# lbcb-sci/GNNome

Hardware: AMD Instinct MI355X
Metric: edges/sec full-graph GatedGCN fwd (higher is better)
Workload: dtype f32

## Files before the change

### gnnome_amd/_lib.py

```python
import ctypes
import os

_HERE = os.path.dirname(os.path.abspath(__file__))
LIB_PATH = os.environ.get("GNNOME_HIP_LIB") or os.path.join(_HERE, "lib", "libgnnome_hip.so")
HEADER_PATH = os.path.join(os.path.dirname(_HERE), "include", "gnnome_hip.h")

_p = ctypes.c_void_p
_i = ctypes.c_int
_l = ctypes.c_int64
_sz = ctypes.c_size_t

SIGNATURES = {
    "gnnome_abi_version": [],
    "gnnome_last_error": [],
    "gnnome_set_tuning": [_i, _i],
    "gnnome_debug_gate_profile": [_p],
    "gnnome_graph_views_workspace_bytes": [_l, _l, ctypes.POINTER(_sz)],
    "gnnome_build_graph_views": [_p, _p, _l, _l, _p, _p, _p, _p, _p, _p, _p, _p, _sz, _p],
    "gnnome_encode_f32": [_p, _l, _i, _p, _p, _p, _i, _p, _p, _i, _p, _p],
    "gnnome_linear_f32": [_p, _l, _i, _i, _p, _i, _p, _i, _p, _i, _p],
    "gnnome_linear_acc_f32": [_p, _l, _i, _i, _p, _i, _p, _i, _p, _i, _p],
    "gnnome_weight_planes_f16": [_p, _i, _i, _i, _p, _p],
    "gnnome_linear_planes_f32": [_p, _l, _i, _i, _p, _p, _i, _p, _i, _p],
    "gnnome_linear_planes_route": [_l, _i, _i, _i],
    "gnnome_edge_gate_f32": [_p, _p, _l, _i, _p, _p, _i, _p, _p, _p, _i, _i, _p, _p, _p],
    "gnnome_edge_gate_encode_f32": [_p, _p, _p, _p, _p, _p, _p, _l, _i, _p, _p, _i, _p, _p, _p, _i, _p, _p, _p],
    "gnnome_linear_ref_f32": [_p, _l, _i, _i, _p, _i, _p, _i, _p, _i, _p],
    "gnnome_edge_gate_ref_f32": [_p, _p, _l, _i, _p, _p, _i, _p, _p, _p, _i, _p, _p, _p, _p, _p, _p, _p, _p, _p, _p],
    "gnnome_node_aggregate_f32": [_p, _i, _l, _p, _p, _p, _i, _p, _p, _p, _p, _p, _p, _i, _p, _i, _p, _p, _p],
    "gnnome_build_node_records": [_p, _p, _p, _p, _p, _l, _p, _p],
    "gnnome_debug_node_records": [_p],
    "gnnome_node_aggregate_range_f32": [_p, _i, _l, _l, _l, _p, _p, _p, _i, _p, _p, _p, _p, _p, _p, _i, _p, _i, _p, _p, _p],
    "gnnome_stream_schedule_sizes": [_l, _l, _i, ctypes.POINTER(_l), ctypes.POINTER(_sz)],
    "gnnome_build_stream_schedule": [_l, _l, _p, _p, _p, _p, _p, _i, _i, _i, _p, _p, _p, _p, _p, _p, _p, _p, _sz, _p],
    "gnnome_node_aggregate_stream_f32": [_p, _i, _l, _l, _p, _p, _p, _i, _p, _p, _p, _p, _p, _p, _i, _p, _p, _p, _i, _i, _i, _p, _p, _p, _p, _p, _p,
                                         _p, _l, _p, _p],
    "gnnome_edge_score_f32": [_p, _l, _i, _i, _p, _p, _i, _p, _p, _p, _p, _i, _p, _p, _p, _p, _p, _p, _p],
    "gnnome_debug_forward_events": [_p, _p, _p, _p, _i],
    "gnnome_model_forward_workspace_bytes": [_l, _l, _i, _i, ctypes.POINTER(_sz)],
    "gnnome_model_forward_f32": [_p, _p, _p, _p, _p, _p, _sz, _p],
    "gnnome_model_forward_buffers_f32": [_p, _p, _p, _p, _p, _p, _p],
    "gnnome_edge_gate_raw_f32": [_p, _p, _l, _i, _p, _p, _i, _p, _p, _p, _i, _p],
    "gnnome_edge_gate_raw_stats_rows": [_i, ctypes.POINTER(_i)],
    "gnnome_edge_gate_raw_stats_f32": [_p, _p, _l, _i, _p, _p, _i, _p, _p, _p, _i, _p, _p, _p],
    "gnnome_edge_gate_raw_stats_x16": [_p, _p, _l, _i, _p, _p, _i, _p, _p, _p, _i, _p, _p, _p],
    "gnnome_edge_gate_bn_f32": [_p, _p, _p, _l, _i, _p, _p, _i, _p, _p, _p, _i, _p, _p, _p],
    "gnnome_edge_gate_bn_x16": [_p, _p, _p, _l, _i, _p, _p, _i, _p, _p, _p, _i, _p, _p, _p],
    "gnnome_node_aggregate_raw_f32": [_p, _i, _l, _i, _p, _p, _p, _i, _p, _p, _p, _p, _p, _p, _p, _p, _p, _p, _p],
    "gnnome_colsum_workspace_bytes": [ctypes.POINTER(_sz)],
    "gnnome_colsum2_f32": [_p, _p, _l, _i, _p, _p, _p, _p, _sz, _p],
    "gnnome_bn_relu_res_f32": [_p, _p, _p, _p, _l, _i, _p, _p],
    "gnnome_bn_relu_res_x16": [_p, _p, _p, _p, _l, _i, _p, _p],
    "gnnome_bn_bwd_stats_f32": [_p, _p, _p, _p, _p, _l, _i, _p, _p, _p, _sz, _p],
    "gnnome_bn_bwd_apply_f32": [_p, _p, _p, _p, _l, _i, _p, _p, _p, _p, _p, _p, _p],
    "gnnome_bn_bwd_apply_tables_f32": [_p, _p, _p, _p, _l, _i, _p, _p, _p, _p, _p, _p, _p, _p, _p, _p, _p, _p, _p, _p, _p, _p],
    "gnnome_ln_relu_res_f32": [_p, _p, _p, _p, _l, _i, _i, _p, _p],
    "gnnome_ln_bwd_f32": [_p, _p, _p, _p, _l, _i, _i, _p, _p, _p, _p, _sz, _p],
    "gnnome_mul23_f32": [_p, _p, _p, _l, _p, _p, _p],
    "gnnome_add_f32": [_p, _p, _l, _p, _p],
    "gnnome_relu_bwd_f32": [_p, _p, _l, _p, _p],
    "gnnome_segment_sum_f32": [_p, _i, _p, _p, _l, _p, _i, _p],
    "gnnome_segment_sum2_f32": [_p, _i, _p, _p, _p, _l, _p, _i, _p, _i, _p],
    "gnnome_segment_sum2_amax_f32": [_p, _i, _p, _p, _p, _l, _p, _i, _p, _i, _p, _p],
    "gnnome_segment_sum2_x16": [_p, _i, _p, _p, _p, _l, _p, _i, _p, _i, _p],
    "gnnome_wgrad_workspace_bytes": [_l, _i, _i, ctypes.POINTER(_sz)],
    "gnnome_wgrad_f32": [_p, _i, _i, _p, _i, _i, _l, _p, _i, _p, _sz, _p],
    "gnnome_wgrad_scaled_f32": [_p, _i, _i, _p, _i, _i, _l, _p, _p, _i, _p, _sz, _p],
    "gnnome_wgrad_x16": [_p, _i, _i, _p, _i, _i, _l, _p, _i, _p, _sz, _p],
    "gnnome_wgrad_blocks_f32": [_p, _i, _i, _i, _p, _i, _i, _l, _p, _i, _p, _p, _sz, _p],
    "gnnome_wgrad_blocks_scaled_f32": [_p, _i, _i, _i, _p, _i, _i, _l, _p, _p, _i, _p, _p, _sz, _p],
    "gnnome_linear_blocks_f32": [_p, _i, _i, _l, _i, _p, _i, _i, _p, _i, _i, _p],
    "gnnome_linear_blocks_scaled_f32": [_p, _i, _i, _l, _i, _p, _i, _i, _p, _p, _i, _i, _p],
    "gnnome_score_tail_bwd_f32": [_p, _p, _p, _l, _i, _p, _p, _p, _p, _p, _p, _p],
    "gnnome_agg_edge_bwd_f32": [_p, _l, _i, _p, _p, _p, _p, _p, _p, _i, _p, _p, _p, _p],
    "gnnome_encode_hidden_f32": [_p, _l, _i, _p, _p, _p, _i, _p, _p],
    "gnnome_gather_rows_f32": [_p, _i, _p, _l, _i, _p, _i, _p],
    "gnnome_scatter_add_rows_f32": [_p, _i, _p, _l, _i, _p, _i, _p],
    "gnnome_closure_workspace_bytes": [ctypes.POINTER(_sz)],
    "gnnome_degree_features_f32": [_p, _p, _l, _i, _p, _p, _sz, _p],
    "gnnome_edge_features_f32": [_p, _p, _l, _p, _p, _sz, _p],
    "gnnome_bn_bwd_dgrad_f32": [_p, _p, _l, _l, _i, _p, _p, _p, _p, _p, _p, _p, _p, _i, _p, _p],
    "gnnome_bn_bwd_dgrad_amax_f32": [_p, _p, _l, _l, _i, _p, _p, _p, _p, _p, _p, _p, _p, _i, _p, _p, _p],
    "gnnome_bn_bwd_dgrad_out_f32": [_p, _p, _p, _l, _l, _i, _p, _p, _p, _p, _p, _p, _p, _p, _i, _p, _p],
    "gnnome_bn_bwd_dgrad_out_amax_f32": [_p, _p, _p, _l, _l, _i, _p, _p, _p, _p, _p, _p, _p, _p, _i, _p, _p, _p],
    "gnnome_bn_bwd_dgrad_x16": [_p, _p, _l, _l, _i, _p, _p, _p, _p, _p, _p, _p, _p, _i, _p, _p],
    "gnnome_bn_bwd_dgrad_out_x16": [_p, _p, _p, _l, _l, _i, _p, _p, _p, _p, _p, _p, _p, _p, _i, _p, _p],
    "gnnome_agg_edge_bwd_stats_f32": [_p, _l, _i, _p, _p, _p, _p, _p, _p, _i, _p, _p, _p, _p, _p, _p, _p, _p, _p, _p, _sz, _p],
    "gnnome_agg_edge_bwd_stats_x16": [_p, _l, _i, _p, _p, _p, _p, _p, _p, _i, _p, _p, _p, _p, _p, _p, _p, _p, _p, _p, _sz, _p],
    "gnnome_agg_bwd_fused_f32": [_p, _l, _l, _i, _p, _p, _p, _p, _p, _p, _i, _p, _p, _p, _p, _p, _p, _p, _p, _p, _p, _p, _p, _p, _p, _p, _p, _sz, _p],
    "gnnome_agg_bwd_fused_x16": [_p, _l, _l, _i, _p, _p, _p, _p, _p, _p, _i, _p, _p, _p, _p, _p, _p, _p, _p, _p, _p, _p, _p, _p, _p, _p, _p, _sz, _p],
    "gnnome_bn_bwd_terms_f32": [_p, _p, _p, _l, _i, _p, _p, _p, _p],
    "gnnome_pack_layer_f32": [_p, _p, _p, _p, _i, _p, _p, _p, _p, _p],
    "gnnome_bn_train_finish_f32": [_p, _p, _p, _l, _i, _p, _p, _p, _p, _p, ctypes.c_float, ctypes.c_float, _i, _p, _p, _p, _p, _p],
    "gnnome_gate_center_f32": [_p, _l, _i, _p, _p, _i, _p, _p, _p, _i, _p, _p],
    "gnnome_greedy_walks_workspace_bytes": [_l, _i, ctypes.POINTER(_sz)],
    "gnnome_greedy_walks": [_p, _p, _p, _p, _p, _p, _p, _l, _p, _p, _p, _i, _p, _p, _l, _p, _p, _p, _p, _p, _p, _p, _sz, _p],
    "gnnome_mark_walk_visited": [_p, _p, _p, _l, _p, _p],
    "gnnome_overlap_workspace_bytes": [ctypes.POINTER(_sz)],
    "gnnome_overlap_edit_distance": [_p, _p, _l, _p, _i, _p, _p, _p, _l, _p, _p, _p, _sz, _p],
    "gnnome_contig_pieces_workspace_bytes": [_l, _l, ctypes.POINTER(_sz)],
    "gnnome_contig_pieces": [_p, _l, _p, _l, _p, _p, _p, _p, _l, _p, _l, _p, _p, _sz, _p],
    "gnnome_contig_spell": [_p, _l, _p, _l, _p, _p, _p, _l, _p, _i, _p, _l, _p],
    "gnnome_edge_labels_workspace_bytes": [_l, _l, ctypes.POINTER(_sz)],
    "gnnome_edge_labels": [_p, _p, _l, _l, _p, _p, _p, _p, _p, _p, _l, _p, _sz, _p],
    "gnnome_cluster_inputs_workspace_bytes": [_l, _l, ctypes.POINTER(_sz)],
    "gnnome_cluster_inputs_f32": [_p, _p, _l, _l, _p, _p, _l, _p, _l, _p, _l, _p, _p, _l, _p, _p, _l, _p, _p, _p, _p, _p, _sz, _p],
    "gnnome_adjacency_support": [_p, _p, _p, _l, _l, _p, _p],
    "gnnome_bfs_levels": [_p, _p, _l, _p, _p, _p, _p, _p, _p, _p],
    "gnnome_hem_propose": [_p, _p, _p, _p, _p, _l, _i, _p, _p],
    "gnnome_kway_gains": [_p, _p, _p, _p, _l, _p, _p, _p],
    "gnnome_greedy_growing_host": [_p, _p, _p, _p, _l, _i, _p],
    "gnnome_edge_loss_f32": [_p, _p, _p, _l, _p, ctypes.c_float, ctypes.c_float, _p, _p, _p, _p, _p, _sz, _p],
    "gnnome_gfa_tile_sizes": [ctypes.POINTER(_i), ctypes.POINTER(_i)],
    "gnnome_gfa_mark": [_p, _l, _p, _p, _p],
    "gnnome_gfa_classify": [_p, _l, _p, _p, _l, _p, _l, _p, _p, _p, _p, _p],
    "gnnome_gfa_names_insert": [_p, _l, _p, _p, _l, _p, _l, _p, _l, _p, _p],
    "gnnome_gfa_links": [_p, _l, _p, _p, _l, _p, _p, _l, _p, _l, _p, _l, _p, _p, _p, _p],
    "gnnome_gfa_pack": [_p, _l, _p, _p, _l, _p, _l, _p],
}

ABI_VERSION = 21


class LayerParams(ctypes.Structure):
    _fields_ = [(n, _p) for n in ("Wcat", "Wcat_planes", "bcat", "W3", "b3", "scale_e", "shift_e", "scale_h", "shift_h")] + [
        ("norm_kind", ctypes.c_int32), ("reference_order", ctypes.c_int32)]


class ModelParams(ctypes.Structure):
    _fields_ = ([(n, ctypes.c_int32) for n in ("hidden", "hidden_ne", "num_layers", "score_hidden", "node_features", "edge_features")]
                + [(n, _p) for n in ("node_W1", "node_b1", "node_W2", "node_b2", "edge_W1", "edge_b1", "edge_W2", "edge_b2")]
                + [("layers_host", ctypes.POINTER(LayerParams)), ("W_nodes", _p), ("W_nodes_planes", _p), ("b_nodes", _p), ("W1e", _p),
                   ("ld_w1e", ctypes.c_int32), ("reserved", ctypes.c_int32), ("W2", _p), ("b2", _p), ("W3", _p), ("b3", _p)])


class Views(ctypes.Structure):
    _fields_ = ([("num_nodes", ctypes.c_int64), ("num_edges", ctypes.c_int64)]
                + [(n, _p) for n in ("in_ptr", "srt_src", "srt_dst", "srt_eid", "out_ptr", "out_pos", "out_dst", "node_gather")]
                + [("transposed", ctypes.c_int32), ("reserved", ctypes.c_int32)])


class ForwardBuffers(ctypes.Structure):
    _fields_ = [("h", _p * 2), ("P", _p), ("e", _p * 2), ("PQ", _p)]


NORM_AFFINE = 0
NORM_LAYER = 1

_lib = None


class GnnomeHipError(RuntimeError):
    pass


def load():
    global _lib
    if _lib is not None:
        return _lib
    if not os.path.isfile(LIB_PATH):
        raise GnnomeHipError(
            f"{LIB_PATH} not found - the HIP extension is not built. Run `make -C gnnome_amd/csrc` "
            "(or __graft_entry__.build()). gnnome_amd has no CPU fallback.")
    lib = ctypes.CDLL(LIB_PATH)
    for name, argtypes in SIGNATURES.items():
        fn = getattr(lib, name)
        fn.argtypes = argtypes
        fn.restype = ctypes.c_char_p if name == "gnnome_last_error" else _i
    got = lib.gnnome_abi_version()
    if got != ABI_VERSION:
        raise GnnomeHipError(f"libgnnome_hip.so ABI {got} != binding ABI {ABI_VERSION}; rebuild")
    _lib = lib
    return lib


def check(rc, what):
    if rc != 0:
        msg = load().gnnome_last_error()
        raise GnnomeHipError(f"{what} failed ({rc}): {msg.decode() if msg else ''}")
```

### gnnome_amd/csrc/common.h

```cpp
#pragma once
#include <hip/hip_runtime.h>
#include <stdint.h>
#include <stdio.h>

#include "../../include/gnnome_hip.h"

namespace gnnome {

void set_error(const char* fmt, ...);

enum { kTuneGateVariant = 0, kTuneGateAblation = 1, kTuneLinearVariant = 2, kTuneGateTileOrder = 3, kTuneGateExperiment = 4, kTuneAggLdsKiB = 5, kTuneAggHubs = 6, kTuneAggVariant = 7, kTuneRefVariant = 8, kTuneOverlapBand = 9, kTuneArith = 10, kTuneCount = 16 };
int tuning(int key);

struct GateEnc {
    const float* e_raw;
    const int32_t* srt_eid;
    const float *W1, *b1, *W2, *b2;
    const float *W23, *b23;
};

struct GateBnBwd {
    const float *a, *c1, *c2, *mean, *rstd, *scale, *shift;
    float* a_out;
    int64_t n_once;
    unsigned* amax_bits = nullptr;
};

struct GateBfArgs {
    const float* e_in;
    float* e_out;
    int64_t E;
    const float* B1h;
    const float* B2h;
    int ldn;
    const int32_t* srt_src;
    const int32_t* srt_dst;
    const float* W3;
    int ldw;
    const float* scale;
    const float* shift;
    float* stats;
    int num_tiles;
    int abl;
    long long* prof;
    int xp;
    int num_cblocks, ld_out;
    GateEnc enc;
    GateBnBwd bnb;
};
int gate_bf_launch(int hidden, int mode, bool enc, const GateBfArgs& args, hipStream_t s, bool x16 = false, int extra = 0);
int gate_stream_launch(const float* e_in, float* e_out, int64_t E, const float* B1h, const float* B2h, int ldn, const int32_t* ss,
                       const int32_t* sd, const float* W3, int ldw, const float* scale, const float* shift, hipStream_t s);

int ws_linear_acc(const float* A, int64_t M, int K, const float* W, int ldw, float* C, hipStream_t s);
int stream_linear_acc_256(const float* A, int64_t M, const float* W, int ldw, float* C, hipStream_t s);
int gate_pl256_launch(int mode, const GateBfArgs& a, hipStream_t s, bool x16 = false);
int gate_f16_launch(int mode, const GateBfArgs& a, int grid, hipStream_t s, bool x16 = false);
int gate_enc256_launch(const GateBfArgs& a, hipStream_t s);
int gate_pl256_stats_rows();
void hub_cache_invalidate();
long long* gate_profile_buffer();
int linear_refm_launch(const float* A, int64_t M, int K, int lda, const float* W, int ldw, const float* bias, int Nout, float* C, int ldc,
                       hipStream_t s);
int gate_refm_launch(int hidden, bool with_enc, const float* e_in, float* e_out, int64_t E, const float* B1h, const float* B2h, int ldn,
                     const int32_t* ss, const int32_t* sd, const float* W3, int ldw, const float* b3, const float* scale, const float* shift,
                     const GateEnc& enc, hipStream_t s);

#define GN_REQUIRE(cond, ...)                 \
    do {                                      \
        if (!(cond)) {                        \
            ::gnnome::set_error(__VA_ARGS__); \
            return GNNOME_EINVAL;             \
        }                                     \
    } while (0)

#define GN_HIP(call)                                                                              \
    do {                                                                                          \
        hipError_t err__ = (call);                                                                \
        if (err__ != hipSuccess) {                                                                \
            ::gnnome::set_error("%s failed: %s (%s:%d)", #call, hipGetErrorString(err__), __FILE__, \
                                __LINE__);                                                        \
            return GNNOME_EHIP;                                                                   \
        }                                                                                         \
    } while (0)

#define GN_LAUNCH_CHECK() GN_HIP(hipGetLastError())

constexpr int kWave = 64;
constexpr int kXcds = 8;
constexpr int kNumCUs = 256;
int persistent_grid();
constexpr float kAggEps = 1e-6f;
constexpr float kNormEps = 1e-5f;

typedef float f32x4 __attribute__((ext_vector_type(4)));
typedef float f32x16 __attribute__((ext_vector_type(16)));

__device__ __forceinline__ unsigned bf16_bits(float x) {
    const unsigned u = __float_as_uint(x);
    return (u + 0x7FFFu + ((u >> 16) & 1u)) >> 16;
}
__device__ __forceinline__ uint2 pack_bf16x4(const f32x4 v) {
    return make_uint2(bf16_bits(v[0]) | (bf16_bits(v[1]) << 16), bf16_bits(v[2]) | (bf16_bits(v[3]) << 16));
}
__device__ __forceinline__ f32x4 unpack_bf16x4(const uint2 p) {
    return f32x4{__uint_as_float(p.x << 16), __uint_as_float(p.x & 0xFFFF0000u), __uint_as_float(p.y << 16),
                 __uint_as_float(p.y & 0xFFFF0000u)};
}
template <bool X16>
__device__ __forceinline__ f32x4 load4_as(const void* base, int64_t off) {
    if (X16) return unpack_bf16x4(*reinterpret_cast<const uint2*>(reinterpret_cast<const uint16_t*>(base) + off));
    return *reinterpret_cast<const f32x4*>(reinterpret_cast<const float*>(base) + off);
}
template <bool X16>
__device__ __forceinline__ void store4_as(void* base, int64_t off, const f32x4 v) {
    if (X16)
        *reinterpret_cast<uint2*>(reinterpret_cast<uint16_t*>(base) + off) = pack_bf16x4(v);
    else
        *reinterpret_cast<f32x4*>(reinterpret_cast<float*>(base) + off) = v;
}


__device__ __forceinline__ int xcd_remap(int bid, int n) {
    const int xcd = bid % kXcds, q = n / kXcds, r = n % kXcds;
    const int base = xcd < r ? xcd * (q + 1) : r * (q + 1) + (xcd - r) * q;
    return base + bid / kXcds;
}

__device__ __forceinline__ float sigmoidf_(float x) { return __builtin_amdgcn_rcpf(1.0f + __expf(-x)); }

__device__ __forceinline__ float relu_keep_nan(float t) { return t < 0.f ? 0.f : t; }

__device__ __forceinline__ void wave_amax_to(unsigned* amax_bits, float v) {
#pragma unroll
    for (int o = 32; o > 0; o >>= 1) v = fmaxf(v, __shfl_xor(v, o));
    if ((threadIdx.x & 63) == 0) {
        const unsigned b = __float_as_uint(v);
        if (b > __hip_atomic_load(amax_bits, __ATOMIC_RELAXED, __HIP_MEMORY_SCOPE_AGENT)) atomicMax(amax_bits, b);
    }
}

__device__ __forceinline__ float half_wave_sum(float v) {
    v += __shfl_xor(v, 1);
    v += __shfl_xor(v, 2);
    v += __shfl_xor(v, 4);
    v += __shfl_xor(v, 8);
    v += __shfl_xor(v, 16);
    return v;
}

}
```

### gnnome_amd/csrc/edge_gate.hip

```cpp
#include "gemm_tile.h"

namespace gnnome {

template <int NB, int NORM>
__global__ __launch_bounds__(kGemmThreads) void k_edge_gate(const float* e_in, float* e_out, int64_t E,
                                                            const float* __restrict__ B1h,
                                                            const float* __restrict__ B2h, int ldn,
                                                            const int32_t* __restrict__ srt_src,
                                                            const int32_t* __restrict__ srt_dst,
                                                            const float* __restrict__ W3, int ldw,
                                                            const float* __restrict__ scale,
                                                            const float* __restrict__ shift, int total_tiles, int norm_width) {
    constexpr int H = 32 * NB;
    __shared__ __attribute__((aligned(16))) float lds[tile_lds_floats<NB>() + 2 * kTileM];
    float* As = lds;
    float* Ws = lds + kTileM * kLdk;
    int* s_src = reinterpret_cast<int*>(lds + tile_lds_floats<NB>());
    int* s_dst = s_src + kTileM;

    const int tid = threadIdx.x, wave = tid >> 6, lane = tid & 63;
    const int tile = xcd_remap(blockIdx.x, total_tiles);
    const int64_t row0 = (int64_t)tile * kTileM;
    const int valid = (int)min((int64_t)kTileM, E - row0);

// ... 489 lines not shown
               "edge_gate: null pointer");
    const int norm_width = (norm_kind >> 8) ? (norm_kind >> 8) : hidden;
    norm_kind &= 0xFF;
    GN_REQUIRE(norm_kind == GNNOME_NORM_AFFINE || norm_kind == GNNOME_NORM_LAYER, "edge_gate: bad norm_kind %d", norm_kind);
    GN_REQUIRE(norm_width >= 1 && norm_width <= hidden && (norm_width == hidden || norm_kind == GNNOME_NORM_LAYER), "edge_gate: bad norm width %d", norm_width);
    GN_REQUIRE(ld_node >= hidden && ldw >= hidden && ldw % 4 == 0, "edge_gate: bad strides");
    GN_REQUIRE(((uintptr_t)e_in % 16 == 0) && ((uintptr_t)W3 % 16 == 0), "edge_gate: e_in and W3 must be 16-byte aligned");
    hipStream_t s = (hipStream_t)stream;
    const int variant = tuning(kTuneGateVariant);
    const bool rows16 = ld_node % 4 == 0 && ((uintptr_t)B1h % 16 == 0) && ((uintptr_t)B2h % 16 == 0);
    const bool persistent_ok = norm_kind == GNNOME_NORM_AFFINE && (hidden == 64 || hidden == 128);
    if (persistent_ok && variant != 1) {
        if ((variant == 0 || variant == 7 || variant == 8) && rows16) {
            GateBfArgs a = {};
            a.e_in = e_in; a.e_out = e_out; a.E = num_edges; a.B1h = B1h; a.B2h = B2h; a.ldn = ld_node; a.srt_src = srt_src;
            a.srt_dst = srt_dst; a.W3 = W3; a.ldw = ldw; a.scale = norm_scale; a.shift = norm_shift;
            return gate_bf_launch(hidden, 0, false, a, s);
        }
        if ((variant == 5 || variant == 6) && rows16) {
            if (hidden == 128)
                return launch_gate_ws<4, 1>(e_in, e_out, num_edges, B1h, B2h, ld_node, srt_src, srt_dst, W3, ldw, norm_scale, norm_shift, s);
            return launch_gate_ws<2, 2>(e_in, e_out, num_edges, B1h, B2h, ld_node, srt_src, srt_dst, W3, ldw, norm_scale, norm_shift, s);
        }
    }
    if (hidden == 256 && norm_kind == GNNOME_NORM_AFFINE && (variant == 0 || variant == 9) && e_in != e_out && ld_node % 4 == 0 &&
        ((uintptr_t)e_out % 16 == 0)) {
        if (variant == 0 && rows16) {
            GateBfArgs a = {};
            a.e_in = e_in; a.e_out = e_out; a.E = num_edges; a.B1h = B1h; a.B2h = B2h; a.ldn = ld_node; a.srt_src = srt_src;
            a.srt_dst = srt_dst; a.W3 = W3; a.ldw = ldw; a.scale = norm_scale; a.shift = norm_shift;
            return gate_pl256_launch(0, a, s);
        }
        return gate_stream_launch(e_in, e_out, num_edges, B1h, B2h, ld_node, srt_src, srt_dst, W3, ldw, norm_scale, norm_shift, s);
    }
    switch (hidden) {
        case 64: return launch_gate<2>(e_in, e_out, num_edges, B1h, B2h, ld_node, srt_src, srt_dst, W3, ldw, norm_kind, norm_scale, norm_shift, s, norm_width);
        case 128: return launch_gate<4>(e_in, e_out, num_edges, B1h, B2h, ld_node, srt_src, srt_dst, W3, ldw, norm_kind, norm_scale, norm_shift, s, norm_width);
        case 256: return launch_gate<8>(e_in, e_out, num_edges, B1h, B2h, ld_node, srt_src, srt_dst, W3, ldw, norm_kind, norm_scale, norm_shift, s, norm_width);
        default: set_error("edge_gate: hidden=%d not in {64,128,256}", hidden); return GNNOME_EINVAL;
    }
}

extern "C" int gnnome_edge_gate_raw_f32(const float* e_in, float* x_out, int64_t num_edges, int hidden, const float* B1h,
                                        const float* B2h, int ld_node, const int32_t* srt_src, const int32_t* srt_dst,
                                        const float* W3, int ldw, void* stream) {
    using namespace gnnome;
    GN_REQUIRE(num_edges >= 0, "edge_gate_raw: negative edge count");
    if (num_edges == 0) return GNNOME_OK;
    GN_REQUIRE(e_in && x_out && x_out != e_in && B1h && B2h && srt_src && srt_dst && W3, "edge_gate_raw: bad pointers");
    GN_REQUIRE(ld_node >= hidden && ldw >= hidden && ldw % 4 == 0, "edge_gate_raw: bad strides");
    GN_REQUIRE(((uintptr_t)e_in % 16 == 0) && ((uintptr_t)W3 % 16 == 0), "edge_gate_raw: e_in and W3 must be 16-byte aligned");
    hipStream_t s = (hipStream_t)stream;
    if (hidden == 256 && tuning(kTuneGateVariant) == 0 && ld_node % 4 == 0 && ((uintptr_t)B1h % 16 == 0) && ((uintptr_t)B2h % 16 == 0) &&
        ((uintptr_t)x_out % 16 == 0)) {
        GateBfArgs a = {};
        a.e_in = e_in; a.e_out = x_out; a.E = num_edges; a.B1h = B1h; a.B2h = B2h; a.ldn = ld_node; a.srt_src = srt_src;
        a.srt_dst = srt_dst; a.W3 = W3; a.ldw = ldw;
        return gate_pl256_launch(1, a, s);
    }
    switch (hidden) {
        case 64: return launch_gate<2>(e_in, x_out, num_edges, B1h, B2h, ld_node, srt_src, srt_dst, W3, ldw, 2, nullptr, nullptr, s);
        case 128: return launch_gate<4>(e_in, x_out, num_edges, B1h, B2h, ld_node, srt_src, srt_dst, W3, ldw, 2, nullptr, nullptr, s);
        case 256: return launch_gate<8>(e_in, x_out, num_edges, B1h, B2h, ld_node, srt_src, srt_dst, W3, ldw, 2, nullptr, nullptr, s);
        default: set_error("edge_gate_raw: hidden=%d not in {64,128,256}", hidden); return GNNOME_EINVAL;
    }
}

extern "C" int gnnome_edge_gate_raw_stats_rows(int hidden, int* rows_host) {
    using namespace gnnome;
    GN_REQUIRE(rows_host && (hidden == 64 || hidden == 128 || hidden == 256), "edge_gate_raw_stats_rows: hidden=%d not in {64,128,256}", hidden);
    if (hidden == 256) {
        *rows_host = gate_pl256_stats_rows();
        return GNNOME_OK;
    }
    *rows_host = (tuning(kTuneGateVariant) == 0 || tuning(kTuneGateVariant) == 8) ? kNumCUs * 8 : kNumCUs * (hidden == 128 ? 1 : 2);
    return GNNOME_OK;
}

static int raw_stats_impl(const float* e_in, void* x_out, int64_t num_edges, int hidden, const float* B1h,
                          const float* B2h, int ld_node, const int32_t* srt_src, const int32_t* srt_dst,
                          const float* W3, int ldw, const float* center, float* stats_partial, void* stream, bool x16) {
    using namespace gnnome;
    GN_REQUIRE(num_edges > 0, "edge_gate_raw_stats: needs at least one edge");
    GN_REQUIRE(e_in && x_out != (const void*)e_in && B1h && B2h && srt_src && srt_dst && W3 && center && stats_partial,
               "edge_gate_raw_stats: bad pointers");
    GN_REQUIRE(x_out || ((hidden == 128 || (hidden == 256 && tuning(kTuneArith) == 0 && !x16)) && tuning(kTuneGateVariant) == 0),
               "edge_gate_raw_stats: x_out may be NULL at hidden = 128 and, as fp16x3 with fp32 storage, 256 (default kernels)");
    GN_REQUIRE(hidden == 64 || hidden == 128 || hidden == 256, "edge_gate_raw_stats: hidden=%d not in {64,128,256}", hidden);
    GN_REQUIRE(ld_node >= hidden && ld_node % 4 == 0 && ldw >= hidden && ldw % 4 == 0, "edge_gate_raw_stats: bad strides");
    GN_REQUIRE(((uintptr_t)e_in % 16 == 0) && ((uintptr_t)W3 % 16 == 0) && ((uintptr_t)B1h % 16 == 0) && ((uintptr_t)B2h % 16 == 0),
               "edge_gate_raw_stats: 16-byte alignment required");
    hipStream_t s = (hipStream_t)stream;
    if (hidden == 256) {
        GateBfArgs a = {};
        a.e_in = e_in; a.e_out = (float*)x_out; a.E = num_edges; a.B1h = B1h; a.B2h = B2h; a.ldn = ld_node; a.srt_src = srt_src;
        a.srt_dst = srt_dst; a.W3 = W3; a.ldw = ldw; a.scale = center; a.stats = stats_partial;
        return gate_pl256_launch(1, a, s, x16);
    }
    if (tuning(kTuneGateVariant) == 0 || tuning(kTuneGateVariant) == 8 || x16) {
        GateBfArgs a = {};
        a.e_in = e_in; a.e_out = (float*)x_out; a.E = num_edges; a.B1h = B1h; a.B2h = B2h; a.ldn = ld_node; a.srt_src = srt_src;
        a.srt_dst = srt_dst; a.W3 = W3; a.ldw = ldw; a.scale = center; a.stats = stats_partial;
        return gate_bf_launch(hidden, 1, false, a, s, x16, x_out == nullptr ? 1 : 0);
    }
    if (hidden == 128)
        return launch_ws_raw_stats<4, 1>(e_in, (float*)x_out, num_edges, B1h, B2h, ld_node, srt_src, srt_dst, W3, ldw, center, stats_partial, s);
    return launch_ws_raw_stats<2, 2>(e_in, (float*)x_out, num_edges, B1h, B2h, ld_node, srt_src, srt_dst, W3, ldw, center, stats_partial, s);
}

extern "C" int gnnome_edge_gate_raw_stats_f32(const float* e_in, float* x_out, int64_t num_edges, int hidden, const float* B1h,
                                              const float* B2h, int ld_node, const int32_t* srt_src, const int32_t* srt_dst,
                                              const float* W3, int ldw, const float* center, float* stats_partial, void* stream) {
    return raw_stats_impl(e_in, x_out, num_edges, hidden, B1h, B2h, ld_node, srt_src, srt_dst, W3, ldw, center, stats_partial, stream, false);
}

extern "C" int gnnome_edge_gate_raw_stats_x16(const float* e_in, uint16_t* x_out, int64_t num_edges, int hidden, const float* B1h,
                                              const float* B2h, int ld_node, const int32_t* srt_src, const int32_t* srt_dst,
                                              const float* W3, int ldw, const float* center, float* stats_partial, void* stream) {
    return raw_stats_impl(e_in, x_out, num_edges, hidden, B1h, B2h, ld_node, srt_src, srt_dst, W3, ldw, center, stats_partial, stream, true);
}

static int gate_bn_impl(const float* e_in, float* e_out, void* x_out, int64_t num_edges, int hidden, const float* B1h, const float* B2h, int ld_node,
                        const int32_t* srt_src, const int32_t* srt_dst, const float* W3, int ldw, const float* scale, const float* shift,
                        void* stream, bool x16) {
    using namespace gnnome;
    GN_REQUIRE(num_edges >= 0, "edge_gate_bn: negative edge count");
    if (num_edges == 0) return GNNOME_OK;
    GN_REQUIRE(e_in && e_out && x_out && x_out != (const void*)e_in && x_out != (void*)e_out && B1h && B2h && srt_src && srt_dst && W3 && scale && shift,
               "edge_gate_bn: bad pointers");
    GN_REQUIRE((hidden == 128 || (hidden == 256 && tuning(kTuneArith) == 0 && !x16)) && tuning(kTuneGateVariant) == 0,
               "edge_gate_bn: built at hidden = 128 and, as fp16x3 with fp32 storage, 256 (default kernels), got %d", hidden);
    GN_REQUIRE(ld_node >= hidden && ld_node % 4 == 0 && ldw >= hidden && ldw % 4 == 0, "edge_gate_bn: bad strides");
    GN_REQUIRE(((uintptr_t)e_in % 16 == 0) && ((uintptr_t)e_out % 16 == 0) && ((uintptr_t)x_out % 16 == 0) && ((uintptr_t)W3 % 16 == 0) &&
                   ((uintptr_t)B1h % 16 == 0) && ((uintptr_t)B2h % 16 == 0), "edge_gate_bn: 16-byte alignment required");
    GateBfArgs a = {};
    a.e_in = e_in; a.e_out = e_out; a.E = num_edges; a.B1h = B1h; a.B2h = B2h; a.ldn = ld_node; a.srt_src = srt_src; a.srt_dst = srt_dst;
    a.W3 = W3; a.ldw = ldw; a.scale = scale; a.shift = shift; a.bnb.a_out = (float*)x_out;
    if (hidden == 256) return gate_pl256_launch(0, a, (hipStream_t)stream, false);
    return gate_bf_launch(hidden, 0, false, a, (hipStream_t)stream, x16, 1);
}

extern "C" int gnnome_edge_gate_bn_f32(const float* e_in, float* e_out, float* x_out, int64_t num_edges, int hidden, const float* B1h,
                                       const float* B2h, int ld_node, const int32_t* srt_src, const int32_t* srt_dst, const float* W3, int ldw,
                                       const float* scale, const float* shift, void* stream) {
    return gate_bn_impl(e_in, e_out, x_out, num_edges, hidden, B1h, B2h, ld_node, srt_src, srt_dst, W3, ldw, scale, shift, stream, false);
}

extern "C" int gnnome_edge_gate_bn_x16(const float* e_in, float* e_out, uint16_t* x_out, int64_t num_edges, int hidden, const float* B1h,
                                       const float* B2h, int ld_node, const int32_t* srt_src, const int32_t* srt_dst, const float* W3, int ldw,
                                       const float* scale, const float* shift, void* stream) {
    return gate_bn_impl(e_in, e_out, x_out, num_edges, hidden, B1h, B2h, ld_node, srt_src, srt_dst, W3, ldw, scale, shift, stream, true);
}

extern "C" int gnnome_edge_gate_encode_f32(const float* e_raw, const int32_t* srt_eid, const float* encW1, const float* encb1,
                                           const float* encW2, const float* encb2, float* e_out, int64_t num_edges, int hidden,
                                           const float* B1h, const float* B2h, int ld_node, const int32_t* srt_src,
                                           const int32_t* srt_dst, const float* W3, int ldw, const float* norm_scale,
                                           const float* norm_shift, void* stream) {
    using namespace gnnome;
    GN_REQUIRE(num_edges >= 0, "edge_gate_encode: negative edge count");
    if (num_edges == 0) return GNNOME_OK;
    GN_REQUIRE(e_raw && srt_eid && encW1 && encb1 && encW2 && encb2 && e_out && B1h && B2h && srt_src && srt_dst && W3 &&
                   norm_scale && norm_shift, "edge_gate_encode: null pointer");
    GN_REQUIRE(hidden == 64 || hidden == 128 || (hidden == 256 && tuning(kTuneArith) == 0 && tuning(kTuneGateVariant) == 0),
               "edge_gate_encode: hidden=%d not in {64,128,256 (default kernels)}", hidden);
    GN_REQUIRE(ld_node % 4 == 0 && ldw % 4 == 0 && ((uintptr_t)B1h % 16 == 0) && ((uintptr_t)B2h % 16 == 0) && ((uintptr_t)W3 % 16 == 0),
               "edge_gate_encode: alignment");
    const GateEnc enc = {e_raw, srt_eid, encW1, encb1, encW2, encb2};
    hipStream_t s = (hipStream_t)stream;
    if (hidden == 256) {
        GN_REQUIRE((uintptr_t)e_out % 16 == 0, "edge_gate_encode: e_out must be 16-byte aligned");
        GateBfArgs a = {};
        a.e_out = e_out; a.E = num_edges; a.B1h = B1h; a.B2h = B2h; a.ldn = ld_node; a.srt_src = srt_src; a.srt_dst = srt_dst;
        a.W3 = W3; a.ldw = ldw; a.scale = norm_scale; a.shift = norm_shift; a.enc = enc;
        return gate_enc256_launch(a, s);
    }
    if (tuning(kTuneGateVariant) == 0 || tuning(kTuneGateVariant) == 7 || tuning(kTuneGateVariant) == 8) {
        GateBfArgs a = {};
        a.e_out = e_out; a.E = num_edges; a.B1h = B1h; a.B2h = B2h; a.ldn = ld_node; a.srt_src = srt_src; a.srt_dst = srt_dst;
        a.W3 = W3; a.ldw = ldw; a.scale = norm_scale; a.shift = norm_shift; a.enc = enc;
        return gate_bf_launch(hidden, 0, true, a, s);
    }
    if (hidden == 128)
        return launch_gate_ws<4, 1>(nullptr, e_out, num_edges, B1h, B2h, ld_node, srt_src, srt_dst, W3, ldw, norm_scale, norm_shift, s, &enc);
    return launch_gate_ws<2, 2>(nullptr, e_out, num_edges, B1h, B2h, ld_node, srt_src, srt_dst, W3, ldw, norm_scale, norm_shift, s, &enc);
}
```

### gnnome_amd/csrc/edge_gate_bf.hip

```cpp
#include "common.h"

namespace gnnome {

typedef __bf16 bf16x8 __attribute__((ext_vector_type(8)));

template <int CB, int RB>
struct GateBF {
    static_assert(CB * RB == 4, "four compute waves");
    static constexpr int H = 32 * CB, TM = 32 * RB, LDK = H + 4, RING = 4, LWAVES = 2;
    static constexpr int NT = 64 * (4 + RING * LWAVES);
    static constexpr int NP = TM * (H / 4) / (64 * LWAVES);
    static constexpr int kSlotFloats = TM * LDK;
    static constexpr int kLdsFloats = RING * 2 * kSlotFloats;
};

__device__ __forceinline__ unsigned lds_addr_bf(const void* p) {
    return (unsigned)(size_t)(__attribute__((address_space(3))) const void*)p;
}
__device__ __forceinline__ void flag_wait_bf(unsigned addr, unsigned want, int nap) {
    unsigned v, spins = 0;
    for (;;) {
        asm volatile("ds_read_b32 %0, %1\n\ts_waitcnt lgkmcnt(0)" : "=v"(v) : "v"(addr) : "memory");
        if (__builtin_amdgcn_readfirstlane(v) >= want) break;
        if (++spins > (1u << 26)) __builtin_trap();
// ... 747 lines not shown
    constexpr int H = 128, TM = 32, RING = 3, LDK = H + 4, TPLD = 48, TPLANE = TM * TPLD, TILEF = TM * LDK;
    constexpr int SLOTB = 3 * TPLANE + 2 * TILEF * 4, NP = 8, RSTEP = 4;
    __shared__ __attribute__((aligned(16))) unsigned char ring[RING * SLOTB];
    __shared__ __attribute__((aligned(16))) float consts[4 * H];
    __shared__ float w1s[32], b1s[16];
    __shared__ unsigned flags[2 * RING];
    const int tid = threadIdx.x, lane = tid & 63;
    const int wave = __builtin_amdgcn_readfirstlane(tid >> 6);
    const unsigned full0 = lds_addr_bf(&flags[0]), done0 = lds_addr_bf(&flags[RING]);
    const int per_xcd = gridDim.x / kXcds;
    const int first = (int)(blockIdx.x % kXcds) * per_xcd + (int)(blockIdx.x / kXcds);
    const int stride = (int)gridDim.x;
    const int n = first < a.num_tiles ? (a.num_tiles - first + stride - 1) / stride : 0;
    if (n <= 0) return;
    auto tile_of = [&](int r) { return first + r * stride; };
    auto tile_valid = [&](int r) { return (int)min((int64_t)TM, a.E - (int64_t)tile_of(r) * TM); };
    if (tid < 4 * H) {
        const int q = tid / H, c = tid % H;
        consts[tid] = q == 0 ? a.scale[c] : q == 1 ? a.shift[c] : q == 2 ? a.enc.b23[c] : a.enc.b2[c];
    }
    if (tid >= 4 * H && tid < 4 * H + 32) w1s[tid - 4 * H] = a.enc.W1[tid - 4 * H];
    if (tid >= 4 * H + 32 && tid < 4 * H + 48) b1s[tid - 4 * H - 32] = a.enc.b1[tid - 4 * H - 32];
    if (tid < 2 * RING) flags[tid] = 0;
    __syncthreads();

    if (wave < 4) {
        const int cl = lane & 31, half = lane >> 5, col = 32 * wave + cl;
        uint4 u1, u2, u3, v1, v2, v3;
        {
            const float* p = a.enc.W23 + col * 16 + 8 * half;
            split3(*reinterpret_cast<const f32x4*>(p), *reinterpret_cast<const f32x4*>(p + 4), u1, u2, u3);
            const float* q = a.enc.W2 + col * 16 + 8 * half;
            split3(*reinterpret_cast<const f32x4*>(q), *reinterpret_cast<const f32x4*>(q + 4), v1, v2, v3);
        }
        auto crow = [](int r) { return (r & 3) + 8 * (r >> 2); };
        const int lane_x = 4 * half * LDK + col;
        const float bxc = consts[2 * H + col], bec = consts[3 * H + col];
        for (int i = 0; i < n; ++i) {
            const int slot = i % RING;
            const unsigned use = (unsigned)(i / RING) + 1u;
            flag_wait_bf(full0 + 4 * slot, 2u * use, 0);
            const unsigned char* tp = ring + slot * SLOTB + cl * TPLD + 16 * half;
            const uint4 c1 = *reinterpret_cast<const uint4*>(tp), c2 = *reinterpret_cast<const uint4*>(tp + TPLANE),
                        c3 = *reinterpret_cast<const uint4*>(tp + 2 * TPLANE);
            f32x16 ax, ae;
#pragma unroll
            for (int r = 0; r < 16; ++r) ax[r] = ae[r] = 0.f;
            ax = __builtin_amdgcn_mfma_f32_32x32x16_bf16(as_bf(c3), as_bf(u1), ax, 0, 0, 0);
            ae = __builtin_amdgcn_mfma_f32_32x32x16_bf16(as_bf(c3), as_bf(v1), ae, 0, 0, 0);
            ax = __builtin_amdgcn_mfma_f32_32x32x16_bf16(as_bf(c1), as_bf(u3), ax, 0, 0, 0);
            ae = __builtin_amdgcn_mfma_f32_32x32x16_bf16(as_bf(c1), as_bf(v3), ae, 0, 0, 0);
            ax = __builtin_amdgcn_mfma_f32_32x32x16_bf16(as_bf(c2), as_bf(u2), ax, 0, 0, 0);
            ae = __builtin_amdgcn_mfma_f32_32x32x16_bf16(as_bf(c2), as_bf(v2), ae, 0, 0, 0);
            ax = __builtin_amdgcn_mfma_f32_32x32x16_bf16(as_bf(c2), as_bf(u1), ax, 0, 0, 0);
            ae = __builtin_amdgcn_mfma_f32_32x32x16_bf16(as_bf(c2), as_bf(v1), ae, 0, 0, 0);
            ax = __builtin_amdgcn_mfma_f32_32x32x16_bf16(as_bf(c1), as_bf(u2), ax, 0, 0, 0);
            ae = __builtin_amdgcn_mfma_f32_32x32x16_bf16(as_bf(c1), as_bf(v2), ae, 0, 0, 0);
            ax = __builtin_amdgcn_mfma_f32_32x32x16_bf16(as_bf(c1), as_bf(u1), ax, 0, 0, 0);
            ae = __builtin_amdgcn_mfma_f32_32x32x16_bf16(as_bf(c1), as_bf(v1), ae, 0, 0, 0);
            float* X = reinterpret_cast<float*>(ring + slot * SLOTB + 3 * TPLANE) + lane_x;
#pragma unroll
            for (int r = 0; r < 16; ++r) {
                X[crow(r) * LDK] = ax[r] + bxc;
                X[TILEF + crow(r) * LDK] = ae[r] + bec;
            }
            flag_bump_bf(done0 + 4 * slot, lane);
        }
    } else {
        const int group = (wave - 4) / 2;
        const int gl = ((wave - 4) % 2) * 64 + lane;
        const int r0 = gl / (H / 4), c4 = gl % (H / 4);
        const int trow = gl >> 2, jq = gl & 3;
        f32x4 g1[NP], g2[NP], gk[NP];
        int si[NP], di[NP], eid = 0;
        float raw0 = 0.f, raw1 = 0.f;
        const unsigned off_row = (unsigned)(r0 * H + 4 * c4);
        auto issue_early = [&](int r) {
            const int64_t row0 = (int64_t)tile_of(r) * TM;
            const int valid = tile_valid(r);
#pragma unroll
            for (int p = 0; p < NP; ++p) {
                const int64_t row = row0 + min(r0 + p * RSTEP, valid - 1);
                si[p] = a.srt_src[row];
                di[p] = a.srt_dst[row];
            }
            eid = a.enc.srt_eid[row0 + min(trow, valid - 1)];
        };
        auto issue_late = [&]() {
            raw0 = a.enc.e_raw[2 * (int64_t)eid];
            raw1 = a.enc.e_raw[2 * (int64_t)eid + 1];
#pragma unroll
            for (int p = 0; p < NP; ++p) {
                g1[p] = *reinterpret_cast<const f32x4*>(a.B1h + (int64_t)si[p] * a.ldn + 4 * c4);
                g2[p] = *reinterpret_cast<const f32x4*>(a.B2h + (int64_t)di[p] * a.ldn + 4 * c4);
            }
        };
        if (group < n) {
            issue_early(group);
            issue_late();
            if (group + RING < n) issue_early(group + RING);
        }
        unsigned char* S = ring + group * SLOTB;
        const float* Xs = reinterpret_cast<const float*>(S + 3 * TPLANE);
        for (int r = group; r < n; r += RING) {
            const unsigned use = (unsigned)(r / RING) + 1u;
            {
                f32x4 t;
#pragma unroll
                for (int j = 0; j < 4; ++j) {
                    const int hu = 4 * jq + j;
                    t[j] = fmaxf(__builtin_fmaf(raw1, w1s[2 * hu + 1], raw0 * w1s[2 * hu]) + b1s[hu], 0.f);
                }
                uint2 p1, p2, p3;
                split4_planes(t, p1, p2, p3);
                unsigned char* d = S + trow * TPLD + 8 * jq;
                *reinterpret_cast<uint2*>(d) = p1;
                *reinterpret_cast<uint2*>(d + TPLANE) = p2;
                *reinterpret_cast<uint2*>(d + 2 * TPLANE) = p3;
            }
#pragma unroll
            for (int p = 0; p < NP; ++p) {
                gk[p] = g1[p] + g2[p];
                asm volatile("" : "+v"(gk[p]));
            }
            flag_bump_bf(full0 + 4 * group, lane);
            if (r + RING < n) issue_late();
            if (r + 2 * RING < n) issue_early(r + 2 * RING);
            flag_wait_bf(done0 + 4 * group, 4u * use, a.xp & 3);
            const int valid = tile_valid(r);
            const f32x4 sc4 = *reinterpret_cast<const f32x4*>(consts + 4 * c4), sh4 = *reinterpret_cast<const f32x4*>(consts + H + 4 * c4);
            float* out = a.e_out + (int64_t)tile_of(r) * TM * H;
#pragma unroll
            for (int pb = 0; pb < NP; pb += 2) {
                f32x4 x[2], e0[2];
#pragma unroll
                for (int u = 0; u < 2; ++u) {
                    x[u] = *reinterpret_cast<const f32x4*>(Xs + (r0 + (pb + u) * RSTEP) * LDK + 4 * c4);
                    e0[u] = *reinterpret_cast<const f32x4*>(Xs + TILEF + (r0 + (pb + u) * RSTEP) * LDK + 4 * c4);
                }
                asm volatile("" : "+v"(x[0]), "+v"(x[1]));
#pragma unroll
                for (int u = 0; u < 2; ++u) {
                    const int p = pb + u, row = r0 + p * RSTEP;
                    f32x4 y;
#pragma unroll
                    for (int j = 0; j < 4; ++j) y[j] = fmaxf((x[u][j] + gk[p][j]) * sc4[j] + sh4[j], 0.f) + e0[u][j];
                    if (row < valid) *reinterpret_cast<f32x4*>(out + (off_row + (unsigned)(p * RSTEP * H))) = y;
                }
            }
        }
    }
}

struct EncFoldScratch {
    float* w23 = nullptr;
};
static EncFoldScratch g_enc_fold[16];

static int launch_enc16(const GateBfArgs& args, hipStream_t s) {
    GateBfArgs a = args;
    const int64_t tiles = (a.E + 31) / 32;
    GN_REQUIRE(tiles < (1ll << 31), "edge_gate: too many tiles");
    a.num_tiles = (int)tiles;
    a.xp = tuning(kTuneGateExperiment);
    int dev = 0;
    GN_HIP(hipGetDevice(&dev));
    GN_REQUIRE(dev >= 0 && dev < 16, "edge_gate_encode: device index %d", dev);
    if (!g_enc_fold[dev].w23) GN_HIP(hipMalloc(&g_enc_fold[dev].w23, sizeof(float) * (128 * 16 + 128)));
    float* w23 = g_enc_fold[dev].w23;
    hipLaunchKernelGGL(k_fold_encoder, dim3((128 * 17 + 3) / 4), dim3(256), 0, s, a.W3, a.ldw, a.enc.W2, a.enc.b2, 128, w23, w23 + 128 * 16);
    GN_LAUNCH_CHECK();
    a.enc.W23 = w23;
    a.enc.b23 = w23 + 128 * 16;
    hipLaunchKernelGGL(k_edge_gate_enc16, dim3(persistent_grid()), dim3(640), 0, s, a);
    GN_LAUNCH_CHECK();
    return GNNOME_OK;
}

static EncFoldScratch g_enc_fold256[16];
int gate_enc256_launch(const GateBfArgs& args, hipStream_t s) {
    GateBfArgs a = args;
    const int64_t tiles = (a.E + 31) / 32;
    GN_REQUIRE(tiles < (1ll << 31), "edge_gate: too many tiles");
    a.num_tiles = (int)tiles;
    a.prof = g_gate_prof;
    int dev = 0;
    GN_HIP(hipGetDevice(&dev));
    GN_REQUIRE(dev >= 0 && dev < 16, "edge_gate_encode: device index %d", dev);
    if (!g_enc_fold256[dev].w23) GN_HIP(hipMalloc(&g_enc_fold256[dev].w23, sizeof(float) * (256 * 16 + 256)));
    float* w23 = g_enc_fold256[dev].w23;
    hipLaunchKernelGGL(k_fold_encoder, dim3((256 * 17 + 3) / 4), dim3(256), 0, s, a.W3, a.ldw, a.enc.W2, a.enc.b2, 256, w23, w23 + 256 * 16);
    GN_LAUNCH_CHECK();
    a.enc.W23 = w23;
    a.enc.b23 = w23 + 256 * 16;
    int g = persistent_grid();
    g -= g % 16;
    return gate_f16_launch(5, a, g < 16 ? 16 : g, s);
}

template <int CB, int RB, int MODE, bool ENC, bool X16 = false>
static int launch_bf(const GateBfArgs& args, hipStream_t s) {
    using P = GateBF<CB, RB>;
    GateBfArgs a = args;
    const int64_t tiles = (a.E + P::TM - 1) / P::TM;
    GN_REQUIRE(tiles < (1ll << 31), "edge_gate: too many tiles");
    a.num_tiles = (int)tiles;
    a.abl = tuning(kTuneGateAblation);
    a.xp = tuning(kTuneGateExperiment);
    a.prof = g_gate_prof;
    if (MODE == 1) GN_HIP(hipMemsetAsync(a.stats, 0, sizeof(float) * kNumCUs * P::RING * P::LWAVES * 2 * P::H, s));
    hipLaunchKernelGGL((k_edge_gate_bf<CB, RB, MODE, ENC, X16>), dim3(persistent_grid()), dim3(P::NT), 0, s, a);
    GN_LAUNCH_CHECK();
    return GNNOME_OK;
}

int gate_bf_launch(int hidden, int mode, bool enc, const GateBfArgs& a, hipStream_t s, bool x16, int extra) {
    const bool planes = hidden == 128 && tuning(kTuneGateVariant) != 8;
    if (extra) {
        GN_REQUIRE(hidden == 128 && !enc && (mode == 0 || mode == 1), "edge-tile kernel: the two-pass training forward is built at hidden = 128");
        if (mode == 1) return x16 ? launch_pl<false, 1, true, 1>(a, s) : launch_pl<false, 1, false, 1>(a, s);
        return x16 ? launch_pl<false, 0, true, 1>(a, s) : launch_pl<false, 0, false, 1>(a, s);
    }
    if (x16) {
        if (mode == 1 && planes) return launch_pl<false, 1, true>(a, s);
        if (mode == 3 && planes) return launch_pl<false, 3, true>(a, s);
        if (mode == 1) return hidden == 128 ? launch_bf<4, 1, 1, false, true>(a, s) : launch_bf<2, 2, 1, false, true>(a, s);
        if (mode == 3) return hidden == 128 ? launch_bf<4, 1, 3, false, true>(a, s) : launch_bf<2, 2, 3, false, true>(a, s);
        set_error("edge-tile kernel: bf16 storage exists for modes 1 and 3 only");
        return GNNOME_EINVAL;
    }
    if (hidden == 128) {
        if (mode == 0 && enc && tuning(kTuneGateVariant) == 0) return launch_enc16(a, s);
        if (mode == 0 && tuning(kTuneGateVariant) != 8) return enc ? launch_pl<true>(a, s) : launch_pl<false>(a, s);
        if (mode == 1 && planes) return launch_pl<false, 1>(a, s);
        if (mode == 3 && planes) return launch_pl<false, 3>(a, s);
        if (mode == 4) return launch_pl<false, 4>(a, s);
        if (mode == 2 && planes) return launch_pl<false, 2>(a, s);
        if (mode == 0) return enc ? launch_bf<4, 1, 0, true>(a, s) : launch_bf<4, 1, 0, false>(a, s);
        if (mode == 3) return launch_bf<4, 1, 3, false>(a, s);
        return mode == 1 ? launch_bf<4, 1, 1, false>(a, s) : launch_bf<4, 1, 2, false>(a, s);
    }
    if (mode == 0) return enc ? launch_bf<2, 2, 0, true>(a, s) : launch_bf<2, 2, 0, false>(a, s);
    if (mode == 3) return launch_bf<2, 2, 3, false>(a, s);
    return mode == 1 ? launch_bf<2, 2, 1, false>(a, s) : launch_bf<2, 2, 2, false>(a, s);
}

}

extern "C" int gnnome_debug_gate_profile(void* counters) {
    gnnome::g_gate_prof = (long long*)counters;
    return GNNOME_OK;
}

static int bn_bwd_dgrad_impl(float* C, const void* X, int64_t rows, int64_t rows_once, int hidden, const float* scale, const float* shift,
                             const float* a, const float* c1, const float* c2, const float* mean, const float* rstd,
                             const float* W, int ldw, void* dxe, void* stream, bool x16, unsigned* amax_bits = nullptr) {
    using namespace gnnome;
    GN_REQUIRE(rows >= 0 && (hidden == 64 || hidden == 128), "bn_bwd_dgrad: hidden=%d not in {64,128}", hidden);
    GN_REQUIRE(rows_once >= 0 && rows_once <= rows, "bn_bwd_dgrad: rows_once=%lld outside [0, rows]", (long long)rows_once);
    if (rows == 0) return GNNOME_OK;
    GN_REQUIRE(C && X && scale && shift && a && c1 && c2 && mean && rstd && W && dxe && dxe != (void*)C && ldw >= hidden && ldw % 4 == 0,
               "bn_bwd_dgrad: bad arguments");
    GN_REQUIRE(((uintptr_t)C % 16 == 0) && ((uintptr_t)X % 16 == 0) && ((uintptr_t)dxe % 16 == 0) && ((uintptr_t)W % 16 == 0),
               "bn_bwd_dgrad: tensors must be 16-byte aligned");
    GateBfArgs g = {};
    g.e_in = (const float*)X; g.e_out = C; g.E = rows; g.B1h = C; g.ldn = hidden; g.W3 = W; g.ldw = ldw;
    g.bnb = GateBnBwd{a, c1, c2, mean, rstd, scale, shift, (float*)dxe, rows_once};
    if (amax_bits != nullptr) {
        GN_REQUIRE(hidden == 128 && tuning(kTuneGateVariant) != 8, "bn_bwd_dgrad_amax: hidden = 128 on the plane-form kernel only");
        GN_HIP(hipMemsetAsync(amax_bits, 0, sizeof(unsigned), (hipStream_t)stream));
        g.bnb.amax_bits = amax_bits;
    }
    return gate_bf_launch(hidden, 3, false, g, (hipStream_t)stream, x16);
}

extern "C" int gnnome_bn_bwd_dgrad_f32(float* C, const float* X, int64_t rows, int64_t rows_once, int hidden, const float* scale, const float* shift,
                                       const float* a, const float* c1, const float* c2, const float* mean, const float* rstd,
                                       const float* W, int ldw, float* dxe, void* stream) {
    return bn_bwd_dgrad_impl(C, X, rows, rows_once, hidden, scale, shift, a, c1, c2, mean, rstd, W, ldw, dxe, stream, false);
}

extern "C" int gnnome_bn_bwd_dgrad_amax_f32(float* C, const float* X, int64_t rows, int64_t rows_once, int hidden, const float* scale,
                                            const float* shift, const float* a, const float* c1, const float* c2, const float* mean,
                                            const float* rstd, const float* W, int ldw, float* dxe, unsigned* amax_bits, void* stream) {
    GN_REQUIRE(amax_bits != nullptr, "bn_bwd_dgrad_amax: null amax_bits");
    return bn_bwd_dgrad_impl(C, X, rows, rows_once, hidden, scale, shift, a, c1, c2, mean, rstd, W, ldw, dxe, stream, false, amax_bits);
}

extern "C" int gnnome_bn_bwd_dgrad_x16(float* C, const uint16_t* X, int64_t rows, int64_t rows_once, int hidden, const float* scale, const float* shift,
                                       const float* a, const float* c1, const float* c2, const float* mean, const float* rstd,
                                       const float* W, int ldw, uint16_t* dxe, void* stream) {
    return bn_bwd_dgrad_impl(C, X, rows, rows_once, hidden, scale, shift, a, c1, c2, mean, rstd, W, ldw, dxe, stream, true);
}

static int bn_bwd_dgrad_out_impl(const float* C_in, float* C_out, const float* X, int64_t rows, int64_t rows_once, int hidden,
                                 const float* scale, const float* shift, const float* a, const float* c1, const float* c2,
                                 const float* mean, const float* rstd, const float* W, int ldw, float* dxe, void* stream, bool x16,
                                 unsigned* amax_bits = nullptr);
extern "C" int gnnome_bn_bwd_dgrad_out_amax_f32(const float* C_in, float* C_out, const float* X, int64_t rows, int64_t rows_once, int hidden,
                                                const float* scale, const float* shift, const float* a, const float* c1, const float* c2,
                                                const float* mean, const float* rstd, const float* W, int ldw, float* dxe, unsigned* amax_bits,
                                                void* stream) {
    GN_REQUIRE(amax_bits != nullptr, "bn_bwd_dgrad_out_amax: null amax_bits");
    return bn_bwd_dgrad_out_impl(C_in, C_out, X, rows, rows_once, hidden, scale, shift, a, c1, c2, mean, rstd, W, ldw, dxe, stream, false, amax_bits);
}
extern "C" int gnnome_bn_bwd_dgrad_out_f32(const float* C_in, float* C_out, const float* X, int64_t rows, int64_t rows_once, int hidden,
                                           const float* scale, const float* shift, const float* a, const float* c1, const float* c2,
                                           const float* mean, const float* rstd, const float* W, int ldw, float* dxe, void* stream) {
    return bn_bwd_dgrad_out_impl(C_in, C_out, X, rows, rows_once, hidden, scale, shift, a, c1, c2, mean, rstd, W, ldw, dxe, stream, false);
}
extern "C" int gnnome_bn_bwd_dgrad_out_x16(const float* C_in, float* C_out, const uint16_t* X, int64_t rows, int64_t rows_once, int hidden,
                                           const float* scale, const float* shift, const float* a, const float* c1, const float* c2,
                                           const float* mean, const float* rstd, const float* W, int ldw, uint16_t* dxe, void* stream) {
    return bn_bwd_dgrad_out_impl(C_in, C_out, (const float*)X, rows, rows_once, hidden, scale, shift, a, c1, c2, mean, rstd, W, ldw, (float*)dxe, stream, true);
}
static int bn_bwd_dgrad_out_impl(const float* C_in, float* C_out, const float* X, int64_t rows, int64_t rows_once, int hidden,
                                 const float* scale, const float* shift, const float* a, const float* c1, const float* c2,
                                 const float* mean, const float* rstd, const float* W, int ldw, float* dxe, void* stream, bool x16,
                                 unsigned* amax_bits) {
    using namespace gnnome;
    GN_REQUIRE(rows >= 0 && hidden == 256, "bn_bwd_dgrad_out: hidden=%d (256 only; 64 / 128 update C in place: gnnome_bn_bwd_dgrad_f32)", hidden);
    if (amax_bits != nullptr) GN_HIP(hipMemsetAsync(amax_bits, 0, sizeof(unsigned), (hipStream_t)stream));
    GN_REQUIRE(rows_once >= 0 && rows_once <= rows, "bn_bwd_dgrad_out: rows_once=%lld outside [0, rows]", (long long)rows_once);
    if (rows == 0) return GNNOME_OK;
    GN_REQUIRE(C_in && C_out && C_out != C_in && X && scale && shift && a && c1 && c2 && mean && rstd && W && dxe && dxe != C_out && dxe != C_in &&
                   ldw >= hidden && ldw % 4 == 0, "bn_bwd_dgrad_out: bad arguments");
    GN_REQUIRE(((uintptr_t)C_in % 16 == 0) && ((uintptr_t)C_out % 16 == 0) && ((uintptr_t)X % 16 == 0) && ((uintptr_t)dxe % 16 == 0) &&
                   ((uintptr_t)W % 16 == 0), "bn_bwd_dgrad_out: tensors must be 16-byte aligned");
    (void)x16;
    GateBfArgs g = {};
    g.e_in = X; g.e_out = C_out; g.E = rows; g.B1h = C_in; g.ldn = hidden; g.W3 = W; g.ldw = ldw;
    g.bnb = GateBnBwd{a, c1, c2, mean, rstd, scale, shift, dxe, rows_once};
    g.bnb.amax_bits = amax_bits;
    return gate_pl256_launch(3, g, (hipStream_t)stream, x16);
}
```

### gnnome_amd/csrc/model_forward.cpp

```cpp
#include "common.h"

namespace gnnome {
namespace {

constexpr size_t kAlign = 256;
size_t rounded(size_t bytes) { return (bytes + kAlign - 1) / kAlign * kAlign; }

struct Workspace {
    size_t h[2], P, e[2], PQ, total;
};
Workspace layout(int64_t n, int64_t e, int hidden, int hs) {
    Workspace w;
    size_t off = 0;
    auto take = [&](size_t bytes) {
        const size_t at = off;
        off += rounded(bytes);
        return at;
    };
    w.h[0] = take(sizeof(float) * n * hidden);
    w.h[1] = take(sizeof(float) * n * hidden);
    w.P = take(sizeof(float) * n * 5 * hidden);
    w.e[0] = take(sizeof(float) * e * hidden);
    w.e[1] = hidden == 256 ? take(sizeof(float) * e * hidden) : w.e[0];
    w.PQ = take(sizeof(float) * n * 2 * hs);
    w.total = off;
    return w;
}

struct ForwardEvents {
    hipEvent_t ev[4] = {nullptr, nullptr, nullptr, nullptr};
    int layer = -1;
};
thread_local ForwardEvents g_events;
int mark(int which, int layer, void* stream) {
    if (layer != g_events.layer || g_events.ev[which] == nullptr) return GNNOME_OK;
    GN_HIP(hipEventRecord(g_events.ev[which], (hipStream_t)stream));
    return GNNOME_OK;
}

int project(const float* A, int64_t M, int K, const float* W, const void* planes, const float* bias, int Nout, float* C, void* stream) {
    if (planes != nullptr && gnnome_linear_planes_route(M, K, Nout, 1)) return gnnome_linear_planes_f32(A, M, K, K, planes, bias, Nout, C, Nout, stream);
    return gnnome_linear_f32(A, M, K, K, W, K, bias, Nout, C, Nout, stream);
}

}
}

extern "C" int gnnome_debug_forward_events(void* gate_start, void* gate_stop, void* aggregate_start, void* aggregate_stop, int layer) {
    using namespace gnnome;
    g_events.ev[0] = (hipEvent_t)gate_start;
    g_events.ev[1] = (hipEvent_t)gate_stop;
    g_events.ev[2] = (hipEvent_t)aggregate_start;
    g_events.ev[3] = (hipEvent_t)aggregate_stop;
    g_events.layer = layer;
    return GNNOME_OK;
}

extern "C" int gnnome_model_forward_workspace_bytes(int64_t num_nodes, int64_t num_edges, int hidden, int score_hidden, size_t* bytes_host) {
    using namespace gnnome;
    GN_REQUIRE(bytes_host && num_nodes >= 0 && num_edges >= 0 && hidden > 0 && score_hidden > 0, "model_forward_workspace_bytes: bad argument");
    *bytes_host = layout(num_nodes, num_edges, hidden, score_hidden).total;
    return GNNOME_OK;
}

#define GN_TRY(call)                       \
    do {                                   \
        const int rc__ = (call);           \
        if (rc__ != GNNOME_OK) return rc__; \
    } while (0)

namespace gnnome {
namespace {
int forward_on(const gnnome_model_params* m, const gnnome_views* g, const float* x, const float* e_raw, float* logits, float* const h[2], float* P,
               float* const eb[2], float* PQ, void* stream);
}
}

static int check_model(const gnnome_model_params* m, const gnnome_views* g) {
    using namespace gnnome;
    GN_REQUIRE(m && g, "model_forward: null parameter block");
    const int H = m->hidden, hs = m->score_hidden, L = m->num_layers;
    GN_REQUIRE(g->num_nodes >= 0 && g->num_edges >= 0 && L >= 0 && (L == 0 || m->layers_host != nullptr), "model_forward: bad sizes");
    GN_REQUIRE(H == 64 || H == 128 || H == 256, "model_forward: hidden=%d (the kernels are built for 64 / 128 / 256; pad narrower models)", H);
    GN_REQUIRE(hs == 32 || hs == 64 || hs == 128, "model_forward: score_hidden=%d (built for 32 / 64 / 128)", hs);
    return GNNOME_OK;
}

extern "C" int gnnome_model_forward_f32(const gnnome_model_params* m, const gnnome_views* g, const float* x, const float* e_raw, float* logits,
                                        void* workspace, size_t workspace_bytes, void* stream) {
    using namespace gnnome;
    GN_TRY(check_model(m, g));
    const int64_t N = g->num_nodes, E = g->num_edges;
    const Workspace ws = layout(N, E, m->hidden, m->score_hidden);
    if (workspace_bytes < ws.total) {
        set_error("model_forward: workspace of %zu bytes, %zu needed", workspace_bytes, ws.total);
        return GNNOME_EWORKSPACE;
    }
    GN_REQUIRE((N == 0 && E == 0) || (workspace != nullptr && (uintptr_t)workspace % kAlign == 0), "model_forward: workspace must be 256-byte aligned");
    GN_REQUIRE(E == 0 || logits != nullptr, "model_forward: null logits");
    char* base = static_cast<char*>(workspace);
    float* h[2] = {reinterpret_cast<float*>(base + ws.h[0]), reinterpret_cast<float*>(base + ws.h[1])};
    float* eb[2] = {reinterpret_cast<float*>(base + ws.e[0]), reinterpret_cast<float*>(base + ws.e[1])};
    return forward_on(m, g, x, e_raw, logits, h, reinterpret_cast<float*>(base + ws.P), eb, reinterpret_cast<float*>(base + ws.PQ), stream);
}

extern "C" int gnnome_model_forward_buffers_f32(const gnnome_model_params* m, const gnnome_views* g, const float* x, const float* e_raw, float* logits,
                                                const gnnome_forward_buffers* b, void* stream) {
    using namespace gnnome;
    GN_TRY(check_model(m, g));
    GN_REQUIRE(b != nullptr, "model_forward_buffers: null buffer block");
    const int64_t N = g->num_nodes, E = g->num_edges;
    GN_REQUIRE(E == 0 || logits != nullptr, "model_forward_buffers: null logits");
    GN_REQUIRE(N == 0 || (b->h[0] && b->h[1] && b->P && b->PQ && b->h[0] != b->h[1]), "model_forward_buffers: node buffers h[0], h[1], P, PQ");
    GN_REQUIRE(E == 0 || (b->e[0] && (m->hidden != 256 || (b->e[1] && b->e[1] != b->e[0]))), "model_forward_buffers: edge buffers e[0] (and e[1] at hidden = 256)");
    for (const void* p : {(const void*)b->h[0], (const void*)b->h[1], (const void*)b->P, (const void*)b->e[0], (const void*)b->e[1], (const void*)b->PQ})
        GN_REQUIRE((uintptr_t)p % 16 == 0, "model_forward_buffers: buffers must be 16-byte aligned");
    float* h[2] = {b->h[0], b->h[1]};
    float* eb[2] = {b->e[0], m->hidden == 256 ? b->e[1] : b->e[0]};
    return forward_on(m, g, x, e_raw, logits, h, b->P, eb, b->PQ, stream);
}

namespace gnnome {
namespace {
int forward_on(const gnnome_model_params* m, const gnnome_views* g, const float* x, const float* e_raw, float* logits, float* const h[2], float* P,
               float* const eb[2], float* PQ, void* stream) {
    const int64_t N = g->num_nodes, E = g->num_edges;
    const int H = m->hidden, hs = m->score_hidden, L = m->num_layers;

    GN_TRY(gnnome_encode_f32(x, N, m->node_features, g->node_gather, m->node_W1, m->node_b1, m->hidden_ne, m->node_W2, m->node_b2, H, h[0], stream));
    const bool wide_ok = tuning(kTuneArith) == 0 && tuning(kTuneGateVariant) == 0;
    const bool fold = L > 0 && m->edge_features == 2 && m->hidden_ne == 16 && (H == 64 || H == 128 || (H == 256 && wide_ok)) &&
                      m->layers_host[0].norm_kind == GNNOME_NORM_AFFINE && E > 0;
    float* e = nullptr;
    if (!fold) {
        e = eb[0];
        GN_TRY(gnnome_encode_f32(e_raw, E, m->edge_features, g->srt_eid, m->edge_W1, m->edge_b1, m->hidden_ne, m->edge_W2, m->edge_b2, H, e, stream));
    }
    int cur = 0;
    for (int i = 0; i < L; ++i) {
        const gnnome_layer_params& lw = m->layers_host[i];
        if (lw.reference_order) GN_TRY(gnnome_linear_ref_f32(h[cur], N, H, H, lw.Wcat, H, lw.bcat, 5 * H, P, 5 * H, stream));
        else GN_TRY(project(h[cur], N, H, lw.Wcat, lw.Wcat_planes, lw.bcat, 5 * H, P, stream));
        const float *A1 = P, *A2 = P + H, *A3 = P + 2 * H, *B1 = P + 3 * H, *B2 = P + 4 * H;
        if (g->transposed) {
            const float* t = A2; A2 = A3; A3 = t;
            t = B1; B1 = B2; B2 = t;
        }
        GN_TRY(mark(0, i, stream));
        if (lw.reference_order) {
            float* out = e ? e : eb[0];
            GN_TRY(gnnome_edge_gate_ref_f32(e, out, E, H, B1, B2, 5 * H, g->srt_src, g->srt_dst, lw.W3, H, lw.b3, lw.scale_e, lw.shift_e,
                                            e ? nullptr : e_raw, e ? nullptr : g->srt_eid, e ? nullptr : m->edge_W1, e ? nullptr : m->edge_b1,
                                            e ? nullptr : m->edge_W2, e ? nullptr : m->edge_b2, stream));
            e = out;
        } else if (e == nullptr) {
            GN_TRY(gnnome_edge_gate_encode_f32(e_raw, g->srt_eid, m->edge_W1, m->edge_b1, m->edge_W2, m->edge_b2, eb[0], E, H, B1, B2, 5 * H, g->srt_src,
                                               g->srt_dst, lw.W3, H, lw.scale_e, lw.shift_e, stream));
            e = eb[0];
        } else if (H == 256 && lw.norm_kind == GNNOME_NORM_AFFINE) {
            float* out = e == eb[0] ? eb[1] : eb[0];
            GN_TRY(gnnome_edge_gate_f32(e, out, E, H, B1, B2, 5 * H, g->srt_src, g->srt_dst, lw.W3, H, lw.norm_kind, lw.scale_e, lw.shift_e, stream));
            e = out;
        } else {
            GN_TRY(gnnome_edge_gate_f32(e, e, E, H, B1, B2, 5 * H, g->srt_src, g->srt_dst, lw.W3, H, lw.norm_kind, lw.scale_e, lw.shift_e, stream));
        }
        GN_TRY(mark(1, i, stream));
        GN_TRY(mark(2, i, stream));
        GN_TRY(gnnome_node_aggregate_f32(e, H, N, A1, A2, A3, 5 * H, g->in_ptr, g->srt_src, g->out_ptr, g->out_pos, g->out_dst, h[cur], H, h[cur ^ 1],
                                         lw.norm_kind, lw.scale_h, lw.shift_h, stream));
        GN_TRY(mark(3, i, stream));
        cur ^= 1;
    }
    GN_TRY(project(h[cur], N, H, m->W_nodes, m->W_nodes_planes, m->b_nodes, 2 * hs, PQ, stream));
    const float *Ps = PQ, *Qd = PQ + hs;
    if (g->transposed) {
        const float* t = Ps; Ps = Qd; Qd = t;
    }
    return gnnome_edge_score_f32(e, E, H, hs, Ps, Qd, 2 * hs, g->srt_src, g->srt_dst, g->srt_eid, m->W1e, m->ld_w1e, m->W2, m->b2, m->W3, m->b3, logits,
                                 nullptr, stream);
}
}
}
```

### gnnome_amd/csrc/node_project.hip

```cpp
#include <cstdlib>

#include "common.h"

#pragma clang diagnostic ignored "-Winline-asm"

namespace gnnome {
namespace {

typedef _Float16 h2_t __attribute__((ext_vector_type(2)));
typedef _Float16 h8_t __attribute__((ext_vector_type(8)));
typedef float f32x2 __attribute__((ext_vector_type(2)));

constexpr float kLoScale = 2048.f, kLoInv = 1.0f / 2048.f;

__device__ __forceinline__ unsigned lds_addr(const void* p) { return (unsigned)(size_t)(__attribute__((address_space(3))) const void*)p; }

__device__ __forceinline__ void dma_piece(const void* src, unsigned voff, unsigned lds) {
    asm volatile("s_mov_b32 m0, %2\n\ts_nop 0\n\tglobal_load_lds_dwordx4 %0, %1" ::"v"(voff), "s"(src), "s"(lds) : "m0");
}

template <int N>
__device__ __forceinline__ void wait_vm() { asm volatile("s_waitcnt vmcnt(%0)" ::"n"(N) : "memory"); }
template <int OFF>
__device__ __forceinline__ void load16_at(f32x4& dst, const float* p) {
    asm volatile("global_load_dwordx4 %0, %1, off offset:%2" : "=v"(dst) : "v"(p), "n"(OFF) : "memory");
}
__device__ __forceinline__ void load4_raw(float& dst, const float* p) { asm volatile("global_load_dword %0, %1, off" : "=v"(dst) : "v"(p) : "memory"); }
__device__ __forceinline__ void landed8(f32x4* r, bool wait) {
    if (wait)
        asm volatile("s_waitcnt vmcnt(0)" : "+v"(r[0]), "+v"(r[1]), "+v"(r[2]), "+v"(r[3]), "+v"(r[4]), "+v"(r[5]), "+v"(r[6]), "+v"(r[7])::"memory");
    else
        asm volatile("" : "+v"(r[0]), "+v"(r[1]), "+v"(r[2]), "+v"(r[3]), "+v"(r[4]), "+v"(r[5]), "+v"(r[6]), "+v"(r[7])::"memory");
}

__device__ __forceinline__ float quad_xor1(float v) { return __int_as_float(__builtin_amdgcn_mov_dpp(__float_as_int(v), 0xB1, 0xF, 0xF, true)); }
__device__ __forceinline__ float quad_xor2(float v) { return __int_as_float(__builtin_amdgcn_mov_dpp(__float_as_int(v), 0x4E, 0xF, 0xF, true)); }
__device__ __forceinline__ void quad_transpose(f32x4& E0, f32x4& E1, f32x4& E2, f32x4& E3, int lane) {
    const bool hi2 = lane & 2, hi1 = lane & 1;
#define GN_SWAP(X, Y, COND, XOR)                       \
    _Pragma("unroll") for (int t = 0; t < 4; ++t) {    \
        const float x = X[t], y = Y[t];                \
        const float py = XOR(y), px = XOR(x);          \
        X[t] = COND ? py : x;                          \
        Y[t] = COND ? y : px;                          \
    }
    GN_SWAP(E0, E2, hi2, quad_xor2) GN_SWAP(E1, E3, hi2, quad_xor2)
    GN_SWAP(E0, E1, hi1, quad_xor1) GN_SWAP(E2, E3, hi1, quad_xor1)
#undef GN_SWAP
}

__device__ __forceinline__ void split8(const f32x4 lo, const f32x4 hi, h8_t& p1, h8_t& p2) {
#pragma unroll
    for (int j = 0; j < 4; ++j) {
        const f32x2 v = j < 2 ? f32x2{lo[2 * j], lo[2 * j + 1]} : f32x2{hi[2 * j - 4], hi[2 * j - 3]};
        const h2_t a = __builtin_convertvector(v, h2_t);
        const f32x2 big = v * kLoScale;
        const f32x2 r = {__builtin_fmaf((float)a[0], -kLoScale, big[0]), __builtin_fmaf((float)a[1], -kLoScale, big[1])};
        const h2_t b = __builtin_convertvector(r, h2_t);
        p1[2 * j] = a[0];
        p1[2 * j + 1] = a[1];
        p2[2 * j] = b[0];
        p2[2 * j + 1] = b[1];
    }
}

}

__host__ __device__ constexpr int frag_col(int i) { return 16 * ((i >> 2) & 1) + 4 * (i >> 3) + (i & 3); }

__global__ __launch_bounds__(256) void k_weight_planes(const float* __restrict__ W, int ldw, int Nout, int K, uint4* __restrict__ planes) {
    const int t = blockIdx.x * 256 + threadIdx.x;
    const int lane = t & 63, ksteps = K / 16, s = (t >> 6) % ksteps, cb = (t >> 6) / ksteps;
    if (cb * 32 >= Nout) return;
    const int col = 32 * cb + frag_col(lane & 31), k = 16 * s + 8 * (lane >> 5);
    const float* w = W + (int64_t)col * ldw + k;
    h8_t p1, p2;
    split8(*reinterpret_cast<const f32x4*>(w), *reinterpret_cast<const f32x4*>(w + 4), p1, p2);
    uint4* dst = planes + ((int64_t)cb * ksteps + s) * 128 + lane;
    dst[0] = __builtin_bit_cast(uint4, p1);
    dst[64] = __builtin_bit_cast(uint4, p2);
}

constexpr int kMaxNout = 1536;
constexpr int kGranuleBytes = 32768;

template <int K, int PROBE = 0>
__global__ __launch_bounds__(256, 2) void k_node_project(const float* __restrict__ A, int64_t M, int lda, const unsigned char* __restrict__ planes,
                                                          const float* __restrict__ bias, int Nout, float* __restrict__ C, int ldc, int64_t total_units,
                                                          long long* prof, int xp) {
    static_assert(K == 64 || K == 128 || K == 256, "K is 64, 128 or 256");
    constexpr int KS = K / 16, GB = K == 64 ? kGranuleBytes / 2 : kGranuleBytes, SPG = GB / 2048, BPG = SPG / KS;
    constexpr int NW = 4, NP = GB / 1024 / NW, NT = 64 * NW, TM = 32 * NW;
    constexpr int NSTORE = (PROBE & 1) ? 0 : 4 * BPG;
    __shared__ __attribute__((aligned(1024))) unsigned char ring[2 * kGranuleBytes];
    __shared__ __attribute__((aligned(16))) float bias_lds[kMaxNout];

    const int tid = threadIdx.x, lane = tid & 63;
    const int wave = __builtin_amdgcn_readfirstlane(tid >> 6);
    long long t_start = 0, t_wait = 0, t_load = 0, r_start = 0;
    if (PROBE & 32) { t_start = __builtin_readcyclecounter(); r_start = __builtin_amdgcn_s_memrealtime(); }
    const int gpt = Nout / (32 * BPG);
    const int share = (gridDim.x & 1) == 0 ? (xp > 0 && xp < 100 ? xp : 55) : 50;
    const int half = gridDim.x / 2;
    const bool second = (gridDim.x & 1) == 0 && (int)blockIdx.x >= half;
    int64_t u0, u1;
    if (share == 50) {
        const int64_t w = xcd_remap(blockIdx.x, gridDim.x);
        u0 = w * total_units / gridDim.x;
        u1 = (w + 1) * total_units / gridDim.x;
    } else {
        const int64_t pr = xcd_remap(blockIdx.x % half, half);
        const int64_t p0 = pr * total_units / half, p1 = (pr + 1) * total_units / half, cut = p0 + (p1 - p0) * share / 100;
        u0 = second ? cut : p0;
        u1 = second ? p1 : cut;
    }
    const int count = (int)(u1 - u0);
    if (count <= 0) return;
    const unsigned ring0 = lds_addr(ring), voff = 16u * lane;
    const unsigned char* mine = planes + (NP * wave) * 1024;

    int g = (int)(u0 % gpt);
    int64_t tile = u0 / gpt;
#pragma unroll
    for (int p = 0; p < NP; ++p) dma_piece(mine + (int64_t)g * GB + p * 1024, voff, ring0 + (NP * wave + p) * 1024);
    {
        float bv[kMaxNout / NT];
#pragma unroll
        for (int i = 0; i < kMaxNout / NT; ++i) {
            bv[i] = 0.f;
            if (bias != nullptr && NT * i < Nout) load4_raw(bv[i], bias + min(tid + NT * i, Nout - 1));
        }
        asm volatile("s_waitcnt vmcnt(0)" ::: "memory");
#pragma unroll
        for (int i = 0; i < kMaxNout / NT; ++i) {
            asm volatile("" : "+v"(bv[i]));
            if (tid + NT * i < Nout) bias_lds[tid + NT * i] = bv[i];
        }
    }

    h8_t a1[KS], a2[KS];
    float* crow[4];
    constexpr bool PREFETCH_ROWS = K <= 128 && !(PROBE & 16);
    f32x4 raw[2 * KS];
    bool ahead = false;
    auto request_rows = [&](f32x4 (&dst)[2 * KS], int64_t t) {
        int64_t row = t * TM + 32 * wave + (lane & 31);
        if (row >= M) row = M - 1;
        const float* arow = A + row * lda + 8 * (lane >> 5);
#define GN_LD(S)                                                         \
    if constexpr (S < KS) {                                              \
        load16_at<64 * S>(dst[2 * (S < KS ? S : 0)], arow);              \
        load16_at<64 * S + 16>(dst[2 * (S < KS ? S : 0) + 1], arow);     \
    }
        GN_LD(0) GN_LD(1) GN_LD(2) GN_LD(3) GN_LD(4) GN_LD(5) GN_LD(6) GN_LD(7)
        GN_LD(8) GN_LD(9) GN_LD(10) GN_LD(11) GN_LD(12) GN_LD(13) GN_LD(14) GN_LD(15)
#undef GN_LD
        static_assert(KS <= 16, "offsets up to 1008 bytes");
    };
    bool fresh = true;
    for (int n = 0; n < count; ++n) {
        long long t_in = 0;
        if (PROBE & 32) t_in = __builtin_readcyclecounter();
        if (fresh) {
            const int64_t row0 = tile * TM + 32 * wave;
            if (!ahead) {
                request_rows(raw, tile);
                landed8(raw, true);
            } else {
                wait_vm<NSTORE>();
                landed8(raw, false);
            }
#pragma unroll
            for (int q = 1; q < KS / 4; ++q) landed8(raw + 8 * q, false);
#pragma unroll
            for (int s = 0; s < KS; ++s) split8(raw[2 * s], raw[2 * s + 1], a1[s], a2[s]);
            ahead = false;
#pragma unroll
            for (int r = 0; r < 4; ++r) {
                int64_t rr = row0 + (lane & 28) + r;
                if (rr >= M) rr = M - 1;
                crow[r] = C + rr * ldc + 16 * (lane >> 5) + 4 * (lane & 3);
            }
            if (PROBE & 32) t_load += __builtin_readcyclecounter() - t_in;
        } else {
            wait_vm<NSTORE>();
        }
        asm volatile("s_waitcnt lgkmcnt(0)\n\ts_barrier" ::: "memory");
        if ((PROBE & 32) && !fresh) t_wait += __builtin_readcyclecounter() - t_in;

        int g_next = g + 1;
        const bool wrap = g_next == gpt;
        if (wrap) g_next = 0;
        if (PREFETCH_ROWS && wrap && n + 1 < count) {
            request_rows(raw, tile + 1);
            ahead = true;
        }
        const unsigned next_slot = ring0 + ((n + 1) & 1) * GB + (NP * wave) * 1024;
        const unsigned char* next_src = mine + (int64_t)g_next * GB;
        const unsigned char* slot = ring + (n & 1) * GB + 16 * lane;
        constexpr int AHEAD = 2;
        h8_t wq1[16], wq2[16];
#pragma unroll
        for (int st = 0; st < AHEAD; ++st) {
            wq1[st] = *reinterpret_cast<const h8_t*>(slot + (2 * st) * 1024);
            wq2[st] = *reinterpret_cast<const h8_t*>(slot + (2 * st + 1) * 1024);
        }
#pragma unroll
        for (int b = 0; b < BPG; ++b) {
            f32x16 accM, accC;
#pragma unroll
            for (int r = 0; r < 16; ++r) accM[r] = accC[r] = 0.f;
#pragma unroll
            for (int s = 0; s < KS; ++s) {
                const int step = b * KS + s;
                constexpr int EVERY = KS / NP;
                if (!(PROBE & 4) && step % EVERY == 0 && step / EVERY < NP) dma_piece(next_src + (step / EVERY) * 1024, voff, next_slot + (step / EVERY) * 1024);
                if (step + AHEAD < SPG) {
                    wq1[step + AHEAD] = *reinterpret_cast<const h8_t*>(slot + (2 * (step + AHEAD)) * 1024);
                    wq2[step + AHEAD] = *reinterpret_cast<const h8_t*>(slot + (2 * (step + AHEAD) + 1) * 1024);
                }
                const h8_t w1 = wq1[step], w2 = wq2[step];
// ... 107 lines not shown
```

### gnnome_amd/engine.py

```python
import torch
import torch.nn.functional as F

from . import ops as hip_ops
from ._lib import NORM_AFFINE, NORM_LAYER
from .graph import views_for


class LayerWeights:
    __slots__ = ("Wcat", "bcat", "W3", "b3", "norm", "scale_e", "shift_e", "scale_h", "shift_h", "ref", "gain_e", "planes")


REFERENCE_ORDER_GAIN = 16.0
ARITHMETIC_MODES = ("auto", "reference", "fast")

BUILT_HIDDEN = (64, 128, 256)
BUILT_SCORE_HIDDEN = (32, 64, 128)


def padded_width(width, built=BUILT_HIDDEN, what="hidden_features"):
    for b in built:
        if width <= b:
            return b
    raise ValueError(f"{what}={width}: the HIP kernels are built for widths up to {built[-1]}")


def _pad(t, *shape):
    if tuple(t.shape) == tuple(shape):
        return t
    out = t.new_zeros(shape)
    out[tuple(slice(0, n) for n in t.shape)] = t
    return out


class Prepared:

    def __init__(self, model, device):
        def dev(t):
            return t.detach().to(device=device, dtype=torch.float32).contiguous()

        arithmetic = getattr(model, "arithmetic", "auto")
        self.device = device
        self.model_hidden = model.linear2_node.out_features
        self.hidden = H = padded_width(self.model_hidden)
        ne = model.linear2_node.in_features
        self.enc_node = tuple(dev(t) for t in (model.linear1_node.weight, model.linear1_node.bias,
                                               _pad(model.linear2_node.weight.detach(), H, ne), _pad(model.linear2_node.bias.detach(), H)))
        self.enc_edge = tuple(dev(t) for t in (model.linear1_edge.weight, model.linear1_edge.bias,
                                               _pad(model.linear2_edge.weight.detach(), H, ne), _pad(model.linear2_edge.bias.detach(), H)))
        self.layers = [prepare_layer(conv, device, arithmetic) for conv in model.gnn.convs]
        self.predictor = prepare_predictor(model.predictor, device)
        weights = [t for lw in self.layers for t in (lw.Wcat, lw.W3)] + [self.predictor["_W1"], self.predictor["W2"]]
        amax = max((float(t.abs().max()) if t.numel() else 0.0) for t in weights) if weights else 0.0
        self.force_bf16x6 = not (amax < hip_ops_fp16_max())
        self.range_verified = self.range_failed = None
        self.block = None


def hip_ops_fp16_max():
    return getattr(hip_ops, "FP16_MAX", 65504.0)


def _inputs_key(views, x, e):
    import weakref
    return (weakref.ref(x), x._version, weakref.ref(e), e._version, weakref.ref(views))


def _same_inputs(key, views, x, e):
    return key is not None and key[0]() is x and key[1] == x._version and key[2]() is e and key[3] == e._version and key[4]() is views


def forward_in_range(ops, prep, views, x, e, xd, ed, check=True):
    bf = getattr(ops, "bf16x6_arithmetic", None)
    if bf is None or getattr(ops, "_TUNING", {}).get(10, 0) == 1:
        return run_stack(ops, prep, views, xd, ed)
    if prep.force_bf16x6 or _same_inputs(prep.range_failed, views, x, e):
        with bf():
            return run_stack(ops, prep, views, xd, ed)
    logits = run_stack(ops, prep, views, xd, ed)
    if not check or _same_inputs(prep.range_verified, views, x, e):
        return logits
    if bool(torch.isfinite(logits).all()):
        prep.range_verified = _inputs_key(views, x, e)
        return logits
    prep.range_failed = _inputs_key(views, x, e)
    with bf():
        return run_stack(ops, prep, views, xd, ed)


def _norm_affine(norm_module, device):
    def dev(t):
        return t.detach().to(device=device, dtype=torch.float32).contiguous()

    if isinstance(norm_module, torch.nn.BatchNorm1d):
        var = norm_module.running_var.detach().float().cpu()
        mean = norm_module.running_mean.detach().float().cpu()
        gamma = norm_module.weight.detach().float().cpu()
        beta = norm_module.bias.detach().float().cpu()
        scale = gamma * (1.0 / torch.sqrt(var + norm_module.eps))
        shift = (beta.double() - mean.double() * scale.double()).float()
        width = padded_width(scale.numel())
        return NORM_AFFINE, dev(_pad(scale, width)), dev(_pad(shift, width))
    if isinstance(norm_module, torch.nn.LayerNorm):
        if abs(norm_module.eps - 1e-5) > 1e-12:
            raise ValueError("LayerNorm eps other than 1e-5 is not supported by the HIP kernels")
        own = int(norm_module.weight.numel())
        width = padded_width(own)
        kind = NORM_LAYER if width == own else (NORM_LAYER | (own << 8))
        return kind, dev(_pad(norm_module.weight.detach(), width)), dev(_pad(norm_module.bias.detach(), width))
    raise TypeError(type(norm_module))


def prepare_layer(conv, device, arithmetic=None):
    def dev(t):
        return t.detach().to(device=device, dtype=torch.float32).contiguous()

    arithmetic = getattr(conv, "arithmetic", "auto") if arithmetic is None else arithmetic
    if arithmetic not in ARITHMETIC_MODES:
        raise ValueError(f"arithmetic must be one of {ARITHMETIC_MODES}, got {arithmetic!r}")
    lw = LayerWeights()
    width = conv.B_3.weight.shape[0]
    hidden = padded_width(width)
    W = lambda lin: _pad(lin.weight.detach(), hidden, hidden)
    b = lambda lin: _pad(lin.bias.detach(), hidden)
    lw.Wcat = dev(torch.cat([W(conv.A_1), W(conv.A_2), W(conv.A_3), W(conv.B_1), W(conv.B_2)], 0))
    lw.W3 = dev(W(conv.B_3))
    lw.b3 = dev(b(conv.B_3))
    lw.norm, lw.scale_e, lw.shift_e = _norm_affine(conv.bn_e, device)
    kind_h, lw.scale_h, lw.shift_h = _norm_affine(conv.bn_h, device)
    assert kind_h == lw.norm
    lw.gain_e = float(lw.scale_e.abs().max()) if lw.norm == NORM_AFFINE and lw.scale_e.numel() else 0.0
    can = hip_ops.reference_order_supported(hidden, lw.norm)
    lw.ref = can and (arithmetic == "reference" or (arithmetic == "auto" and lw.gain_e > REFERENCE_ORDER_GAIN))
    planes_ok = getattr(hip_ops, "planes_supported", None)
    lw.planes = hip_ops.weight_planes(lw.Wcat) if (not lw.ref and planes_ok is not None and planes_ok(hidden, 5 * hidden)
                                                   and lw.Wcat.is_cuda) else None
    if lw.ref:
        lw.bcat = dev(torch.cat([b(conv.A_1), b(conv.A_2), b(conv.A_3), b(conv.B_1), b(conv.B_2)], 0))
    else:
        lw.bcat = dev(torch.cat([b(conv.A_1), b(conv.A_2), b(conv.A_3), b(conv.B_1), b(conv.B_2) + b(conv.B_3)], 0))
    return lw


def prepare_predictor(pred, device):
    def dev(t):
        return t.detach().to(device=device, dtype=torch.float32).contiguous()

    hs_model, h3 = pred.W1.weight.shape
    width = h3 // 3
    if pred.W2.out_features != 32 or pred.W3.in_features != 32 or pred.W3.out_features != 1:
        raise ValueError("ScorePredictor tail must be hs -> 32 -> 1 (score_predictor.py:9-10)")
    hidden, hs = padded_width(width), padded_width(hs_model, BUILT_SCORE_HIDDEN, "hidden_edge_scores")
    W1 = dev(torch.cat([_pad(pred.W1.weight.detach()[:, i * width:(i + 1) * width], hs, hidden) for i in range(3)], 1))
    b1 = _pad(pred.W1.bias.detach(), hs)
    W_nodes = torch.cat([W1[:, :hidden], W1[:, hidden:2 * hidden]], 0).contiguous()
    b_nodes = torch.cat([torch.zeros_like(b1), b1])
    planes_ok = getattr(hip_ops, "planes_supported", None)
    planes = (hip_ops.weight_planes(W_nodes) if planes_ok is not None and W_nodes.is_cuda and planes_ok(hidden, 2 * hs) and 2 * hs >= 128 else None)
    return {
        "planes": planes,
        "hidden": hidden, "hs": hs, "model_hidden": width, "W_nodes": W_nodes, "b_nodes": dev(b_nodes), "W1_e": W1[:, 2 * hidden:],
        "W2": dev(_pad(pred.W2.weight.detach(), 32, hs)), "b2": dev(pred.W2.bias),
        "W3": dev(pred.W3.weight.reshape(-1)), "b3": dev(pred.W3.bias.reshape(-1)), "_W1": W1,
    }


class _StateProbe:

    __slots__ = ("device", "arithmetic", "slots", "modules")

    def __init__(self, module, device):
        self.device, self.arithmetic = str(device), getattr(module, "arithmetic", "auto")
        self.slots, self.modules = [], []
        for sub in module.modules():
            self.modules.append((sub._modules, len(sub._modules)))
            for table in (sub._parameters, sub._buffers):
                for name, t in table.items():
                    if t is not None:
                        self.slots.append((table, name, t, t._version, t.data_ptr()))

    def unchanged(self, module, device):
        if str(device) != self.device or getattr(module, "arithmetic", "auto") != self.arithmetic:
            return False
        for table, count in self.modules:
            if len(table) != count:
                return False
        for table, name, t, version, ptr in self.slots:
            if table.get(name) is not t or t._version != version or t.data_ptr() != ptr:
                return False
        return True


def prepared_for(module, device, build):
    cached = module.__dict__.get("_gnnome_prepared")
    if cached is None or not cached[0].unchanged(module, device):
        probe = _StateProbe(module, device)
        cached = (probe, build(module, device))
        module.__dict__["_gnnome_prepared"] = cached
    return cached[1]


def compute_device(*tensors):
    for t in tensors:
        if t.is_cuda:
            return t.device
    if not torch.cuda.is_available():
        raise RuntimeError("gnnome_amd runs on an MI355X only: no HIP device is visible and there is no CPU fallback")
    return torch.device("cuda", torch.cuda.current_device())


def _refuse_training(module):
    if module.training and (torch.is_grad_enabled() or any(isinstance(m, torch.nn.BatchNorm1d) for m in module.modules())):
        raise NotImplementedError("train mode is supported through SymGatedGCNModel.forward only; call .eval() for the "
                                  "layer-level API")
    if torch.is_grad_enabled() and any(p.requires_grad for p in module.parameters()):
        raise NotImplementedError("gnnome_amd layer-level forward is inference-only: its outputs carry no autograd history - wrap the "
                                  "call in torch.no_grad() (or freeze the parameters), or train through SymGatedGCNModel.forward")



def gate_update(ops, lw, views, e, B1, B2, scratch=None):
    if scratch is not None and e.shape[1] == 256 and lw.norm == 0 and getattr(ops, "edge_gate_out_of_place_at_256", False):
        spare = scratch.get("e_spare")
        if spare is None or spare.shape != e.shape or spare.device != e.device:
            spare = torch.empty_like(e)
        ops.edge_gate(e, B1, B2, views, lw.W3, lw.norm, lw.scale_e, lw.shift_e, out=spare)
        scratch["e_spare"] = e
        return spare
    ops.edge_gate(e, B1, B2, views, lw.W3, lw.norm, lw.scale_e, lw.shift_e)
    return e


def project(ops, lw, h, out=None):
    if lw.ref:
        return ops.linear_ref(h, lw.Wcat, lw.bcat, out=out)
    return ops.linear(h, lw.Wcat, lw.bcat, out=out, planes=lw.planes)


def gate(ops, lw, views, e, B1, B2, raw_edges=None, scratch=None):
    if lw.ref:
        return ops.edge_gate_ref(e, B1, B2, views, lw.W3, lw.b3, lw.scale_e, lw.shift_e, raw_edges=raw_edges)
    if e is None:
        return ops.edge_gate_encode(raw_edges[0], raw_edges[1], B1, B2, views, lw.W3, lw.scale_e, lw.shift_e)
    return gate_update(ops, lw, views, e, B1, B2, scratch)


def aggregate_then_project(ops, lw, views, e, A1, A2, A3, h, then):
    n = h.shape[0]
    side = ops.side_stream(h.device)
    main = torch.cuda.current_stream(h.device)
    h_out = torch.empty_like(h)
    P_next = torch.empty((n, then.width), dtype=torch.float32, device=h.device)
    bounds = [n * i // PIPELINE_CHUNKS // 32 * 32 for i in range(PIPELINE_CHUNKS)] + [n]
    for lo, hi in zip(bounds[:-1], bounds[1:]):
        ops.node_aggregate(e, A1, A2, A3, views, h, lw.norm, lw.scale_h, lw.shift_h, node_range=(lo, hi), out=h_out)
        done = torch.cuda.Event()
        done.record(main)
        with torch.cuda.stream(side):
            side.wait_event(done)
            then(h_out[lo:hi], out=P_next[lo:hi])
    main.wait_stream(side)
    return h_out, P_next


import os as _os
ONE_CALL_FORWARD = _os.environ.get("GNNOME_ONE_CALL_FORWARD", "1") != "0"
PIPELINE_CHUNKS = 1
PIPELINE_MIN_NODES = 1 << 15


class _Projection:

    def __init__(self, fn, W, b):
        self.fn, self.W, self.b, self.width = fn, W, b, W.shape[0]

    def __call__(self, rows, out=None):
        return self.fn(rows, self.W, self.b, out=out)


def layer_projection(ops, lw):
    if lw.ref:
        return _Projection(ops.linear_ref, lw.Wcat, lw.bcat)
    return _Projection(lambda rows, W, b, out=None: ops.linear(rows, W, b, out=out, planes=lw.planes), lw.Wcat, lw.bcat)


def layer_step(ops, lw, views, h, e, n_out=None, raw_edges=None, scratch=None, P=None, then=None):
    H = h.shape[1]
    if P is None:
        P = project(ops, lw, h)
    A1, A2, A3, B1, B2 = (P[:, i * H:(i + 1) * H] for i in range(5))
    if views.transposed:
        A2, A3, B1, B2 = A3, A2, B2, B1
    e = gate(ops, lw, views, e, B1, B2, raw_edges, scratch)
    if then is not None:
        h_new, P_next = aggregate_then_project(ops, lw, views, e, A1, A2, A3, h, then)
        return h_new, e, P_next
    return ops.node_aggregate(e, A1, A2, A3, views, h, lw.norm, lw.scale_h, lw.shift_h, num_nodes_out=n_out), e, None


def encode_nodes(ops, views, x, enc):
    gather = getattr(views, "node_gather", None)
    if gather is None:
        return ops.encode(x, *enc)
    return ops.encode(x, *enc, gather=gather, rows=views.num_nodes)


def encode_edges(ops, prep, views, e_raw):
    fuse = getattr(ops, "can_fuse_edge_encoder", None)
    if prep.layers and fuse is not None and fuse(e_raw, prep.enc_edge, prep.hidden, prep.layers[0].norm, prep.layers[0].Wcat):
        return None
    return ops.encode(e_raw, *prep.enc_edge, gather=views.srt_eid, rows=views.num_edges)


def predictor_projection(ops, pw):
    return _Projection(lambda rows, W, b, out=None: ops.linear(rows, W, b, out=out, planes=pw.get("planes")), pw["W_nodes"], pw["b_nodes"])


def score_step(ops, pw, views, h, e, logits, n_edges=None, PQ=None):
    hs = pw["hs"]
    if PQ is None:
        PQ = ops.linear(h, pw["W_nodes"], pw["b_nodes"], planes=pw.get("planes"))
    Ps, Qd = PQ[:, :hs], PQ[:, hs:]
    if views.transposed:
        Ps, Qd = Qd, Ps
    return ops.edge_score(e, Ps, Qd, views, pw["W1_e"], pw["W2"], pw["b2"], pw["W3"], pw["b3"], logits, num_edges=n_edges)


def run_stack(ops, prep, views, x, e_raw, exchange=None, n_own=None, n_score=None, logits=None):
    pipelined = (exchange is None and n_own is None and getattr(ops, "side_stream", None) is not None and PIPELINE_CHUNKS > 1
                 and views.num_nodes >= PIPELINE_MIN_NODES)
    one_call = getattr(ops, "model_forward", None)
    if (ONE_CALL_FORWARD and one_call is not None and exchange is None and n_own is None and n_score is None and not pipelined
            and not getattr(ops, "STREAM_AGGREGATE", False) and isinstance(views, ops.GraphViews) and x.is_cuda and x.is_contiguous()
            and e_raw.is_contiguous()):
        block = getattr(prep, "block", None)
        if block is None:
            block = prep.block = ops.ModelBlock(prep)
        with ops.node_records_for(views, prep.hidden):
            return one_call(block, views, x, e_raw, logits)
    h = encode_nodes(ops, views, x, prep.enc_node)
    e = encode_edges(ops, prep, views, e_raw)
    scratch = {}
    P = None
    for i, lw in enumerate(prep.layers):
        if exchange is not None:
            h = exchange(h)
        then = None
        if pipelined:
            then = layer_projection(ops, prep.layers[i + 1]) if i + 1 < len(prep.layers) else predictor_projection(ops, prep.predictor)
        h, e, P = layer_step(ops, lw, views, h, e, n_out=n_own, raw_edges=(e_raw, prep.enc_edge), scratch=scratch, P=P, then=then)
    if exchange is not None:
        h = exchange(h)
    if logits is None:
        logits = torch.empty(views.num_edges if n_score is None else n_score, dtype=torch.float32, device=h.device)
    score_step(ops, prep.predictor, views, h, e, logits, n_edges=n_score, PQ=P)
    return logits



def model_forward(model, graph, x, e):
    if model.training:
        from .train import train_forward
        return train_forward(model, graph, x, e).to(x.device)
    out_device = x.device
    device = compute_device(x, e)
    prep = prepared_for(model, device, Prepared)
    views = views_for(graph, device, node_order=getattr(model, "node_order", "input"))
    if x.shape[0] != views.num_nodes or e.shape[0] != views.num_edges:
        raise ValueError(f"x has {x.shape[0]} rows for {views.num_nodes} nodes, e has {e.shape[0]} rows for {views.num_edges} edges")
    with torch.no_grad():
        xd = x.detach().to(device=device, dtype=torch.float32).contiguous()
        ed = e.detach().to(device=device, dtype=torch.float32).contiguous()
        logits = forward_in_range(hip_ops, prep, views, x, e, xd, ed, check=getattr(model, "range_check", True))
    views.check_range()
    return logits.unsqueeze(1).to(out_device)


def layer_forward_edge_id_order(conv, g, h, e):
    _refuse_training(conv)
    out_device = h.device
    device = compute_device(h, e)
    lw = prepared_for(conv, device, prepare_layer)
    views = views_for(g, device)
    with torch.no_grad():
        hd = h.detach().to(device=device, dtype=torch.float32).contiguous()
        ed = e.detach().to(device=device, dtype=torch.float32).contiguous()
        width, hidden = hd.shape[1], lw.W3.shape[0]
        if hidden != width:
            hd, ed = F.pad(hd, (0, hidden - width)), F.pad(ed, (0, hidden - width))
        es = hip_ops.gather_rows(ed, views.srt_eid)
        if views.node_gather is not None:
            hd = hip_ops.gather_rows(hd, views.node_gather)
        h_new, _, _ = layer_step(hip_ops, lw, views, hd, es)
        if views.node_perm is not None:
            h_new = h_new.index_select(0, views.node_perm)
        e_new = torch.empty_like(es)
        e_new[views.srt_eid.long()] = es
        if hidden != width:
            h_new, e_new = h_new[:, :width].contiguous(), e_new[:, :width].contiguous()
        h_new = F.dropout(h_new, conv.dropout, training=conv.training)
    views.check_range()
    return h_new.to(out_device), e_new.to(out_device)


def score_forward_edge_id_order(pred, graph, x, e):
    _refuse_training(pred)
    out_device = x.device
    device = compute_device(x, e)
    pw = prepared_for(pred, device, prepare_predictor)
    views = views_for(graph, device)
    with torch.no_grad():
        xd = x.detach().to(device=device, dtype=torch.float32).contiguous()
        ed = e.detach().to(device=device, dtype=torch.float32).contiguous()
        if pw["hidden"] != pw["model_hidden"]:
            xd, ed = (F.pad(t, (0, pw["hidden"] - pw["model_hidden"])) for t in (xd, ed))
        es = hip_ops.gather_rows(ed, views.srt_eid)
        if views.node_gather is not None:
            xd = hip_ops.gather_rows(xd, views.node_gather)
        logits = torch.empty(views.num_edges, dtype=torch.float32, device=device)
        score_step(hip_ops, pw, views, xd, es, logits)
    views.check_range()
    return logits.unsqueeze(1).to(out_device)
```

### gnnome_amd/ops.py

```python
import ctypes

import torch

from . import _lib
from ._lib import NORM_AFFINE, NORM_LAYER


def _ptr(t):
    return ctypes.c_void_p(t.data_ptr() if t is not None and t.numel() > 0 else None)


def _stream(device):
    return ctypes.c_void_p(torch.cuda.current_stream(device).cuda_stream)


_SIDE_STREAMS = {}


def side_stream(device):
    s = _SIDE_STREAMS.get(device.index)
    if s is None:
        s = _SIDE_STREAMS[device.index] = torch.cuda.Stream(device=device, priority=-1)
    return s

# ... 123 lines not shown
        r.transposed = not self.transposed
        r._c_block = None
        return r


import os as _os
STREAM_AGGREGATE = "auto" if _os.environ.get("GNNOME_STREAM_AGGREGATE", "off").lower() in ("1", "on", "auto", "true") else False
STREAM_MIN_EDGES = 400_000
STREAM_MAX_FAR = 0.20
STREAM_ROWS_PER_CHUNK = 2048
STREAM_ROWS_PER_STEP = 16
STREAM_SLOTS = 62


class StreamSchedule:

    __slots__ = ("chunks", "chunk_node", "chunk_steps", "steps", "edge_meta", "node_pend", "pend_nodes", "counters", "num_pending",
                 "num_far", "num_overflow", "max_live", "max_steps", "total_steps", "far_fraction", "usable", "why")

    def __init__(self, views, chunks=None, slots=None):
        lib = _lib.load()
        dev, n, e = views.device, views.num_nodes, views.num_edges
        self.usable, self.why = False, ""
        if e == 0 or n == 0:
            self.why = "empty graph"
            return
        cus = torch.cuda.get_device_properties(dev).multi_processor_count
        self.chunks = int(chunks) if chunks else max(2 * cus, -(-e // STREAM_ROWS_PER_CHUNK))
        slots = STREAM_SLOTS if slots is None else int(slots)
        cap, scratch = ctypes.c_int64(0), ctypes.c_size_t(0)
        _lib.check(lib.gnnome_stream_schedule_sizes(n, e, STREAM_ROWS_PER_STEP, ctypes.byref(cap), ctypes.byref(scratch)), "stream_schedule_sizes")
        mk = lambda k: torch.empty(k, dtype=torch.int32, device=dev)
        self.chunk_node, self.chunk_steps = mk(self.chunks + 1), mk(self.chunks)
        self.steps = torch.empty((int(cap.value), 4), dtype=torch.int32, device=dev)
        self.edge_meta = torch.empty(e, dtype=torch.uint8, device=dev)
        self.node_pend, self.pend_nodes, self.counters = mk(n), mk(n), mk(8)
        ws = torch.empty(int(scratch.value), dtype=torch.uint8, device=dev)
        with _on(dev):
            _lib.check(lib.gnnome_build_stream_schedule(n, e, _ptr(views.in_ptr), _ptr(views.srt_src), _ptr(views.out_ptr), _ptr(views.out_pos),
                                                        _ptr(views.out_dst), self.chunks, STREAM_ROWS_PER_STEP, slots, _ptr(self.chunk_node),
                                                        _ptr(self.chunk_steps), _ptr(self.steps), _ptr(self.edge_meta), _ptr(self.node_pend),
                                                        _ptr(self.pend_nodes), _ptr(self.counters), _ptr(ws), ws.numel(), _stream(dev)),
                       "build_stream_schedule")
            ws.record_stream(torch.cuda.current_stream(dev))
        c = self.counters.tolist()
        self.num_pending, self.num_far, self.num_overflow, self.max_live, self.max_steps = c[0], c[1], c[2], c[3], c[4]
        self.total_steps = int(self.chunk_steps.sum())
        self.far_fraction = self.num_far / e
        if self.far_fraction > STREAM_MAX_FAR:
            self.why = f"{self.far_fraction:.0%} of the rows are far: the numbering has no locality (or the graph is too small for its chunks)"
        elif self.max_steps > 4 * (self.total_steps // self.chunks + 16):
            self.why = f"a chunk of {self.max_steps} steps against {self.total_steps // self.chunks} on average: a hub"
        else:
            self.usable = True


def stream_schedule_for(views, e_rows, num_nodes_out, node_range, norm_kind):
    if (not STREAM_AGGREGATE or norm_kind != NORM_AFFINE or node_range is not None or views.num_edges < STREAM_MIN_EDGES
            or e_rows != views.num_edges or (num_nodes_out is not None and num_nodes_out != views.num_nodes) or not hasattr(views, "stream_schedule")):
        return None
    sched = views.stream_schedule()
    return sched if sched.usable else None


edge_gate_out_of_place_at_256 = True


_TUNING = {}


def set_tuning(key, value):
    _lib.check(_lib.load().gnnome_set_tuning(int(key), int(value)), "set_tuning")
    _TUNING[int(key)] = int(value)


FP16_MAX = 65504.0


class bf16x6_arithmetic:

    def __enter__(self):
        self.prev = _TUNING.get(10, 0)
        if self.prev != 1:
            set_tuning(10, 1)
        return self

    def __exit__(self, *exc):
        if self.prev != 1:
            set_tuning(10, self.prev)


def encode(x, W1, b1, W2, b2, gather=None, rows=None):
    lib = _lib.load()
    x, _ = _rows(x.contiguous(), "encode.in")
    hidden, hidden_ne = W2.shape[0], W1.shape[0]
    rows = int(x.shape[0] if rows is None else rows)
    out = torch.empty((rows, hidden), dtype=torch.float32, device=x.device)
    with _on(x.device):
        _lib.check(lib.gnnome_encode_f32(_ptr(x), rows, x.shape[1], _ptr(gather), _ptr(W1), _ptr(b1), hidden_ne, _ptr(W2),
                                         _ptr(b2), hidden, _ptr(out), _stream(x.device)), "encode_f32")
    return out


def planes_supported(K, Nout):
    return K in (64, 128, 256) and Nout % (32 if K == 256 else 64) == 0 and 0 < Nout <= 1536


def weight_planes(W):
    lib = _lib.load()
    W, ldw = _rows(W, "weight_planes.W")
    Nout, K = W.shape
    planes = torch.empty(Nout * K * 2, dtype=torch.float16, device=W.device)
    with _on(W.device):
        _lib.check(lib.gnnome_weight_planes_f16(_ptr(W), ldw, Nout, K, _ptr(planes), _stream(W.device)), "weight_planes_f16")
    return planes


def _planes_route(A, lda, W, ldw, out, ldc, accumulate, given):
    return (not accumulate and lda % 4 == 0 and ldw % 4 == 0 and ldc % 4 == 0 and A.data_ptr() % 16 == 0 and W.data_ptr() % 16 == 0
            and out.data_ptr() % 16 == 0 and A.data_ptr() != out.data_ptr()
            and _lib.load().gnnome_linear_planes_route(A.shape[0], A.shape[1], W.shape[0], 1 if given else 0) == 1)


def linear(A, W, bias, out=None, accumulate=False, planes=None):
    lib = _lib.load()
    A, lda = _rows(A, "linear.A")
    W, ldw = _rows(W, "linear.W")
    M, K = A.shape
    Nout = W.shape[0]
    if out is None:
        out = torch.empty((M, Nout), dtype=torch.float32, device=A.device)
    out, ldc = _rows(out, "linear.out")
    if _planes_route(A, lda, W, ldw, out, ldc, accumulate, planes is not None):
        if planes is None:
            planes = weight_planes(W)
        with _on(A.device):
            _lib.check(lib.gnnome_linear_planes_f32(_ptr(A), M, K, lda, _ptr(planes), _ptr(bias), Nout, _ptr(out), ldc, _stream(A.device)),
                       "linear_planes_f32")
        return out
    with _on(A.device):
        fn = lib.gnnome_linear_acc_f32 if accumulate else lib.gnnome_linear_f32
        _lib.check(fn(_ptr(A), M, K, lda, _ptr(W), ldw, _ptr(bias), Nout, _ptr(out), ldc, _stream(A.device)), "linear_f32")
    return out


def _dptr(t):
    return t.data_ptr() if t is not None and t.numel() > 0 else None


class ModelBlock:

    def __init__(self, prep):
        pw = prep.predictor
        self.keep = [prep.enc_node, prep.enc_edge, prep.layers, pw]
        n = len(prep.layers)
        self.layers = (_lib.LayerParams * max(n, 1))()
        for lp, lw in zip(self.layers, prep.layers):
            for name in ("Wcat", "bcat", "W3", "b3", "scale_e", "shift_e", "scale_h", "shift_h"):
                t = getattr(lw, name)
                if not (t.is_cuda and t.dtype == torch.float32 and t.is_contiguous()):
                    raise TypeError(f"model_forward: layer tensor {name} must be a contiguous CUDA float32 tensor")
                setattr(lp, name, _dptr(t))
            lp.Wcat_planes = _dptr(lw.planes)
            lp.norm_kind, lp.reference_order = int(lw.norm), int(bool(lw.ref))
        m = self.params = _lib.ModelParams()
        m.hidden, m.num_layers, m.score_hidden = prep.hidden, n, pw["hs"]
        (W1, b1, W2, b2), (V1, c1, V2, c2) = prep.enc_node, prep.enc_edge
        m.hidden_ne, m.node_features, m.edge_features = W1.shape[0], W1.shape[1], V1.shape[1]
        if V1.shape[0] != W1.shape[0]:
            raise ValueError("model_forward: the two encoders share hidden_ne (models/full_graph.py:13-16)")
        m.node_W1, m.node_b1, m.node_W2, m.node_b2 = (_dptr(t) for t in (W1, b1, W2, b2))
        m.edge_W1, m.edge_b1, m.edge_W2, m.edge_b2 = (_dptr(t) for t in (V1, c1, V2, c2))
        m.layers_host = ctypes.cast(self.layers, ctypes.POINTER(_lib.LayerParams))
        W1e = pw["W1_e"]
        if W1e.stride(1) != 1:
            raise ValueError("model_forward: predictor W1's edge block must have contiguous rows")
        m.W_nodes, m.W_nodes_planes, m.b_nodes = _dptr(pw["W_nodes"]), _dptr(pw.get("planes")), _dptr(pw["b_nodes"])
        m.W1e, m.ld_w1e = _dptr(W1e), W1e.stride(0)
        m.W2, m.b2, m.W3, m.b3 = (_dptr(pw[k]) for k in ("W2", "b2", "W3", "b3"))


def _views_block(views):
    blk = getattr(views, "_c_block", None)
    if blk is None:
        blk = _lib.Views()
        blk.num_nodes, blk.num_edges = views.num_nodes, views.num_edges
        for name in ("in_ptr", "srt_src", "srt_dst", "srt_eid", "out_ptr", "out_pos", "out_dst"):
            setattr(blk, name, _dptr(getattr(views, name)))
        blk.node_gather = _dptr(getattr(views, "node_gather", None))
        blk.transposed = int(bool(views.transposed))
        try:
            views._c_block = blk
        except AttributeError:
            pass
    return blk


_WS_BYTES = {}


FORWARD_BUFFERS = _os.environ.get("GNNOME_FORWARD_BUFFERS", "separate")


NODE_RECORDS_MAX_HIDDEN = int(_os.environ.get("GNNOME_NODE_RECORDS", "64"))


class node_records_for:

    def __init__(self, views, hidden):
        self.on = (0 < hidden <= NODE_RECORDS_MAX_HIDDEN and isinstance(views, GraphViews) and views.num_nodes > 0 and views.num_edges > 0
                   and not torch.cuda.is_current_stream_capturing())
        self.views = views

    def __enter__(self):
        if self.on:
            _lib.check(_lib.load().gnnome_debug_node_records(_ptr(self.views.node_records())), "debug_node_records")
        return self

    def __exit__(self, *exc):
        if self.on:
            _lib.load().gnnome_debug_node_records(None)


def model_forward(block, views, x, e_raw, logits=None):
    lib = _lib.load()
    dev = x.device
    m = block.params
    n, e, H, hs = views.num_nodes, views.num_edges, m.hidden, m.score_hidden
    if logits is None:
        logits = torch.empty(e, dtype=torch.float32, device=dev)
    if FORWARD_BUFFERS == "block":
        key = (n, e, H, hs)
        need = _WS_BYTES.get(key)
        if need is None:
            nb = ctypes.c_size_t(0)
            _lib.check(lib.gnnome_model_forward_workspace_bytes(n, e, H, hs, ctypes.byref(nb)), "model_forward_workspace_bytes")
            need = _WS_BYTES[key] = nb.value
        ws = torch.empty(max(need, 256), dtype=torch.uint8, device=dev)
        with _on(dev):
            _lib.check(lib.gnnome_model_forward_f32(ctypes.byref(m), ctypes.byref(_views_block(views)), _ptr(x), _ptr(e_raw), _ptr(logits), _ptr(ws), need,
                                                    _stream(dev)), "model_forward_f32")
        return logits
    shapes = {"h0": (n, H), "h1": (n, H), "P": (n, 5 * H), "PQ": (n, 2 * hs), "e0": (e, H)}
    if H == 256:
        shapes["e1"] = (e, H)
    vb = _views_block(views)

    def run(t):
        bufs = _lib.ForwardBuffers()
        bufs.h[0], bufs.h[1], bufs.P, bufs.PQ = t["h0"].data_ptr(), t["h1"].data_ptr(), t["P"].data_ptr(), t["PQ"].data_ptr()
        bufs.e[0], bufs.e[1] = t["e0"].data_ptr(), (t["e1"].data_ptr() if "e1" in t else None)
        _lib.check(lib.gnnome_model_forward_buffers_f32(ctypes.byref(m), ctypes.byref(vb), _ptr(x), _ptr(e_raw), _ptr(logits), ctypes.byref(bufs),
                                                        _stream(dev)), "model_forward_buffers_f32")

    with _on(dev):
        run(_placed_buffers(dev, shapes, run))
    return logits


TUNE_PLACEMENT = _os.environ.get("GNNOME_TUNE_PLACEMENT", "1") != "0"
PLACEMENT_AFTER_USES = 3
PLACEMENT_CANDIDATES = 4
PLACEMENT_MIN_TOTAL, PLACEMENT_MAX_BUFFER = 64 << 20, 1 << 30
PLACEMENT_KEPT = 3


class _Placed:
    __slots__ = ("uses", "tried", "bufs", "log")

    def __init__(self):
        self.uses, self.tried, self.bufs, self.log = 0, False, None, None


_PLACED = {}


def _placed_buffers(dev, shapes, run):
    mk = lambda name: torch.empty((max(shapes[name][0], 1), shapes[name][1]), dtype=torch.float32, device=dev)
    sizes = [max(r, 1) * c * 4 for r, c in shapes.values()]
    if not TUNE_PLACEMENT or sum(sizes) < PLACEMENT_MIN_TOTAL or max(sizes) >= PLACEMENT_MAX_BUFFER or torch.cuda.is_current_stream_capturing():
        return {name: mk(name) for name in shapes}
    stream = torch.cuda.current_stream(dev)
    key = (dev.index, stream.cuda_stream) + tuple(sorted(shapes.items()))
    st = _PLACED.get(key)
    if st is None:
        st = _PLACED[key] = _Placed()
    if st.bufs is not None:
        return st.bufs
    st.uses += 1
    cur = {name: mk(name) for name in shapes}
    free = torch.cuda.mem_get_info(dev)[0]
    if st.tried or st.uses < PLACEMENT_AFTER_USES or free < 2 * (PLACEMENT_CANDIDATES + 1) * sum(sizes):
        return cur
    st.tried = True

    def time_of(t):
        run(t)
        t0, t1 = torch.cuda.Event(enable_timing=True), torch.cuda.Event(enable_timing=True)
        t0.record(stream)
        run(t)
        run(t)
        t1.record(stream)
        t1.synchronize()
        return t0.elapsed_time(t1) / 2

    for _ in range(3):
        run(cur)
    best, log, rejected = time_of(cur), [], []
    log.append(("start", best))
    for group in (tuple(k for k in ("e0", "e1") if k in shapes), ("P",), ("h0", "h1", "PQ")):
        for _ in range(PLACEMENT_CANDIDATES):
            cand = dict(cur)
            for name in group:
                cand[name] = mk(name)
            t = time_of(cand)
            log.append((group, t))
            if t < best * 0.997:
                rejected.extend(cur[name] for name in group)
                cur, best = cand, t
            else:
                rejected.extend(cand[name] for name in group)
    st.bufs, st.log = cur, log
    del rejected, cand
    try:
        torch.cuda.empty_cache()
    except RuntimeError:
        pass
    kept = [k for k, v in _PLACED.items() if v.bufs is not None]
    for k in kept[:-PLACEMENT_KEPT]:
        _PLACED[k].bufs = None
    return cur


def edge_gate(e, B1h, B2h, views, W3, norm_kind, scale, shift, out=None, num_edges=None):
    lib = _lib.load()
    e, _ = _rows(e, "edge_gate.e")
    B1h, ldn = _rows(B1h, "edge_gate.B1h")
    B2h, ldn2 = _rows(B2h, "edge_gate.B2h")
    assert ldn == ldn2 and e.is_contiguous()
    W3, ldw = _rows(W3, "edge_gate.W3")
    out = e if out is None else out
    E = int(e.shape[0] if num_edges is None else num_edges)
    with _on(e.device):
        _lib.check(lib.gnnome_edge_gate_f32(_ptr(e), _ptr(out), E, e.shape[1], _ptr(B1h), _ptr(B2h), ldn,
                                            _ptr(views.srt_src), _ptr(views.srt_dst), _ptr(W3), ldw, norm_kind, _ptr(scale),
                                            _ptr(shift), _stream(e.device)), "edge_gate_f32")
    return out


def can_fuse_edge_encoder(e_raw, enc, hidden, norm_kind, B1h):
    widths = (64, 128, 256) if _TUNING.get(10, 0) == 0 and _TUNING.get(0, 0) == 0 else (64, 128)
    return (e_raw.dim() == 2 and e_raw.shape[1] == 2 and enc[0].shape == (16, 2) and hidden in widths
            and norm_kind == NORM_AFFINE and e_raw.shape[0] > 0 and B1h.stride(0) % 4 == 0 and B1h.data_ptr() % 16 == 0)


def edge_gate_encode(e_raw, enc, B1h, B2h, views, W3, scale, shift):
    lib = _lib.load()
    e_raw = _dense(e_raw, "edge_gate_encode.e_raw")
    B1h, ldn = _rows(B1h, "edge_gate_encode.B1h")
    B2h, _ = _rows(B2h, "edge_gate_encode.B2h")
    W3, ldw = _rows(W3, "edge_gate_encode.W3")
    E, H = views.num_edges, W3.shape[0]
    out = torch.empty((E, H), dtype=torch.float32, device=e_raw.device)
    W1, b1, W2, b2 = enc
    with _on(e_raw.device):
        _lib.check(lib.gnnome_edge_gate_encode_f32(_ptr(e_raw), _ptr(views.srt_eid), _ptr(W1), _ptr(b1), _ptr(W2), _ptr(b2),
                                                   _ptr(out), E, H, _ptr(B1h), _ptr(B2h), ldn, _ptr(views.srt_src),
                                                   _ptr(views.srt_dst), _ptr(W3), ldw, _ptr(scale), _ptr(shift),
                                                   _stream(e_raw.device)), "edge_gate_encode_f32")
    return out


def linear_ref(A, W, bias, out=None):
    lib = _lib.load()
    A, lda = _rows(A, "linear_ref.A")
    W, ldw = _rows(W, "linear_ref.W")
    M, K = A.shape
    Nout = W.shape[0]
    if out is None:
        out = torch.empty((M, Nout), dtype=torch.float32, device=A.device)
    out, ldc = _rows(out, "linear_ref.out")
    with _on(A.device):
        _lib.check(lib.gnnome_linear_ref_f32(_ptr(A), M, K, lda, _ptr(W), ldw, _ptr(bias), Nout, _ptr(out), ldc, _stream(A.device)),
                   "linear_ref_f32")
    return out


def reference_order_supported(hidden, norm_kind, B1h=None):
    return hidden in (64, 128, 256) and norm_kind == NORM_AFFINE


def edge_gate_ref(e, B1h, B2h, views, W3, b3, scale, shift, raw_edges=None, num_edges=None):
    lib = _lib.load()
    B1h, ldn = _rows(B1h, "edge_gate_ref.B1h")
    B2h, ldn2 = _rows(B2h, "edge_gate_ref.B2h")
    W3, ldw = _rows(W3, "edge_gate_ref.W3")
    assert ldn == ldn2
    H = W3.shape[0]
    if e is None:
        e_raw, (W1, b1, W2, b2) = raw_edges
        e_raw = _dense(e_raw, "edge_gate_ref.e_raw")
        E = views.num_edges if num_edges is None else int(num_edges)
        out = torch.empty((views.num_edges, H), dtype=torch.float32, device=e_raw.device)
        enc = (_ptr(e_raw), _ptr(views.srt_eid), _ptr(W1), _ptr(b1), _ptr(W2), _ptr(b2))
        e_in = _ptr(None)
    else:
        e = _dense(e, "edge_gate_ref.e")
        E = int(e.shape[0] if num_edges is None else num_edges)
        out, e_in = e, _ptr(e)
        enc = (_ptr(None),) * 6
    with _on(out.device):
        _lib.check(lib.gnnome_edge_gate_ref_f32(e_in, _ptr(out), E, H, _ptr(B1h), _ptr(B2h), ldn, _ptr(views.srt_src),
                                                _ptr(views.srt_dst), _ptr(W3), ldw, _ptr(b3), _ptr(scale), _ptr(shift), *enc,
                                                _stream(out.device)), "edge_gate_ref_f32")
    return out


def node_aggregate(e, A1h, A2h, A3h, views, h_in, norm_kind, scale, shift, num_nodes_out=None, node_range=None, out=None):
    lib = _lib.load()
    A1h, ldn = _rows(A1h, "node_aggregate.A1h")
    A2h, l2 = _rows(A2h, "node_aggregate.A2h")
    A3h, l3 = _rows(A3h, "node_aggregate.A3h")
    h_in, ldh = _rows(h_in, "node_aggregate.h_in")
    assert ldn == l2 == l3
    hidden = h_in.shape[1]
    n_out = int(h_in.shape[0] if num_nodes_out is None else num_nodes_out)
    h_out = torch.empty((h_in.shape[0], hidden), dtype=torch.float32, device=h_in.device) if out is None else out
    assert h_out.is_contiguous() and h_out.shape == (h_in.shape[0], hidden) and h_out.dtype == torch.float32
    sched = None
    if STREAM_AGGREGATE and getattr(views, "num_nodes", None) == h_in.shape[0]:
        sched = stream_schedule_for(views, e.shape[0], num_nodes_out, node_range, norm_kind)
    with _on(h_in.device):
        if sched is not None:
            pend = torch.empty((max(sched.num_pending, 1), 3, hidden), dtype=torch.float32, device=h_in.device)
            _lib.check(lib.gnnome_node_aggregate_stream_f32(_ptr(e), hidden, n_out, views.num_edges, _ptr(A1h), _ptr(A2h), _ptr(A3h), ldn, _ptr(views.in_ptr),
                                                            _ptr(views.srt_src), _ptr(views.out_ptr), _ptr(views.out_pos), _ptr(views.out_dst),
                                                            _ptr(h_in), ldh, _ptr(h_out), _ptr(scale), _ptr(shift), sched.chunks,
                                                            STREAM_ROWS_PER_STEP, STREAM_SLOTS, _ptr(sched.chunk_node), _ptr(sched.chunk_steps),
                                                            _ptr(sched.steps), _ptr(sched.edge_meta), _ptr(sched.node_pend), _ptr(sched.pend_nodes),
                                                            _ptr(sched.counters), sched.num_pending, _ptr(pend), _stream(h_in.device)),
                       "node_aggregate_stream_f32")
        elif node_range is None:
            _lib.check(lib.gnnome_node_aggregate_f32(_ptr(e), hidden, n_out, _ptr(A1h), _ptr(A2h), _ptr(A3h), ldn,
                                                     _ptr(views.in_ptr), _ptr(views.srt_src), _ptr(views.out_ptr),
                                                     _ptr(views.out_pos), _ptr(views.out_dst), _ptr(h_in), ldh, _ptr(h_out),
                                                     norm_kind, _ptr(scale), _ptr(shift), _stream(h_in.device)),
                       "node_aggregate_f32")
        else:
            assert out is not None, "node_aggregate(node_range=...) writes rows of a caller-owned `out`"
            _lib.check(lib.gnnome_node_aggregate_range_f32(_ptr(e), hidden, n_out, int(node_range[0]), int(node_range[1]), _ptr(A1h),
                                                           _ptr(A2h), _ptr(A3h), ldn, _ptr(views.in_ptr), _ptr(views.srt_src),
                                                           _ptr(views.out_ptr), _ptr(views.out_pos), _ptr(views.out_dst), _ptr(h_in),
                                                           ldh, _ptr(h_out), norm_kind, _ptr(scale), _ptr(shift),
                                                           _stream(h_in.device)), "node_aggregate_range_f32")
    return h_out


def edge_score(e, Ps, Qd, views, W1e, W2, b2, W3, b3, logits, num_edges=None, scatter_to_edge_id=True, z1_out=None):
    lib = _lib.load()
    e, _ = _rows(e, "edge_score.e")
    Ps, ldn = _rows(Ps, "edge_score.Ps")
    Qd, ldn2 = _rows(Qd, "edge_score.Qd")
    assert ldn == ldn2 and e.is_contiguous()
    W1e, ldw1 = _rows(W1e, "edge_score.W1e")
    E = int(e.shape[0] if num_edges is None else num_edges)
    eid = views.srt_eid if scatter_to_edge_id else None
    with _on(e.device):
        _lib.check(lib.gnnome_edge_score_f32(_ptr(e), E, e.shape[1], W2.shape[1], _ptr(Ps), _ptr(Qd), ldn,
                                             _ptr(views.srt_src), _ptr(views.srt_dst), _ptr(eid), _ptr(W1e), ldw1,
                                             _ptr(W2), _ptr(b2), _ptr(W3), _ptr(b3), _ptr(logits), _ptr(z1_out),
                                             _stream(e.device)), "edge_score_f32")
    return logits


def gather_rows(table, idx, out=None):
    lib = _lib.load()
    table, ld_in = _rows(table, "gather_rows.in")
    _i32(idx, "gather_rows.idx")
    rows, width = int(idx.numel()), table.shape[1]
    if out is None:
        out = torch.empty((rows, width), dtype=torch.float32, device=table.device)
    out, ld_out = _rows(out, "gather_rows.out")
    with _on(table.device):
        _lib.check(lib.gnnome_gather_rows_f32(_ptr(table), ld_in, _ptr(idx), rows, width, _ptr(out), ld_out,
                                              _stream(table.device)), "gather_rows_f32")
    return out


def scatter_add_rows(src, idx, out):
    src, ld_in = _rows(src, "scatter_add_rows.in")
    out, ld_out = _rows(out, "scatter_add_rows.out")
    _i32(idx, "scatter_add_rows.idx")
    if int(idx.numel()) != src.shape[0] or src.shape[1] != out.shape[1]:
        raise ValueError("scatter_add_rows: shape mismatch")
    _call("gnnome_scatter_add_rows_f32", src.device, _ptr(src), ld_in, _ptr(idx), int(idx.numel()), src.shape[1], _ptr(out), ld_out)
    return out



def _call(name, device, *args):
    lib = _lib.load()
    with _on(device):
        _lib.check(getattr(lib, name)(*args, _stream(device)), name)


def _dense(t, name):
    _f32(t, name)
    if not t.is_contiguous():
        raise ValueError(f"{name}: expected a contiguous tensor")
    return t


def edge_gate_raw(e, B1h, B2h, views, W3):
    e = _dense(e, "edge_gate_raw.e")
    B1h, ldn = _rows(B1h, "edge_gate_raw.B1h")
    B2h, _ = _rows(B2h, "edge_gate_raw.B2h")
    W3, ldw = _rows(W3, "edge_gate_raw.W3")
    out = torch.empty_like(e)
# ... 561 lines not shown
```

### include/gnnome_hip.h

```cpp
#ifndef GNNOME_HIP_H
#define GNNOME_HIP_H

#include <stddef.h>
#include <stdint.h>

#ifdef __cplusplus
extern "C" {
#endif

#define GNNOME_ABI_VERSION 21

#define GNNOME_OK 0
#define GNNOME_EINVAL (-1)
#define GNNOME_EHIP (-2)
#define GNNOME_EWORKSPACE (-3)

#define GNNOME_NORM_AFFINE 0
#define GNNOME_NORM_LAYER 1
#define GNNOME_NORM_LAYER_OVER(w) (GNNOME_NORM_LAYER | ((w) << 8))

int gnnome_abi_version(void);
const char* gnnome_last_error(void);

int gnnome_set_tuning(int key, int value);

int gnnome_debug_gate_profile(void* counters);

int gnnome_graph_views_workspace_bytes(int64_t num_nodes, int64_t num_edges, size_t* bytes_host);
int gnnome_build_graph_views(const int32_t* src, const int32_t* dst, int64_t num_nodes, int64_t num_edges,
                             int32_t* in_ptr, int32_t* srt_src, int32_t* srt_dst, int32_t* srt_eid,
                             int32_t* out_ptr, int32_t* out_pos, int32_t* out_dst, void* workspace,
                             size_t workspace_bytes, void* stream);

int gnnome_encode_f32(const float* in, int64_t rows, int in_features, const int32_t* gather,
                      const float* W1, const float* b1, int hidden_ne, const float* W2, const float* b2,
                      int hidden, float* out, void* stream);

int gnnome_linear_f32(const float* A, int64_t M, int K, int lda, const float* W, int ldw, const float* bias,
                      int Nout, float* C, int ldc, void* stream);
int gnnome_linear_acc_f32(const float* A, int64_t M, int K, int lda, const float* W, int ldw, const float* bias,
                          int Nout, float* C, int ldc, void* stream);

int gnnome_weight_planes_f16(const float* W, int ldw, int Nout, int K, void* planes, void* stream);
int gnnome_linear_planes_f32(const float* A, int64_t M, int K, int lda, const void* planes, const float* bias, int Nout, float* C,
                             int ldc, void* stream);
int gnnome_linear_planes_route(int64_t M, int K, int Nout, int given_planes);

int gnnome_edge_gate_f32(const float* e_in, float* e_out, int64_t num_edges, int hidden,
                         const float* B1h, const float* B2h, int ld_node, const int32_t* srt_src,
                         const int32_t* srt_dst, const float* W3, int ldw, int norm_kind,
                         const float* norm_scale, const float* norm_shift, void* stream);

int gnnome_edge_gate_encode_f32(const float* e_raw, const int32_t* srt_eid, const float* encW1, const float* encb1,
                                const float* encW2, const float* encb2, float* e_out, int64_t num_edges, int hidden,
                                const float* B1h, const float* B2h, int ld_node, const int32_t* srt_src,
                                const int32_t* srt_dst, const float* W3, int ldw, const float* norm_scale,
                                const float* norm_shift, void* stream);

int gnnome_linear_ref_f32(const float* A, int64_t M, int K, int lda, const float* W, int ldw, const float* bias, int Nout,
                          float* C, int ldc, void* stream);
int gnnome_edge_gate_ref_f32(const float* e_in, float* e_out, int64_t num_edges, int hidden, const float* B1h,
                             const float* B2h, int ld_node, const int32_t* srt_src, const int32_t* srt_dst, const float* W3,
                             int ldw, const float* b3, const float* norm_scale, const float* norm_shift, const float* e_raw,
                             const int32_t* srt_eid, const float* encW1, const float* encb1, const float* encW2,
                             const float* encb2, void* stream);

int gnnome_node_aggregate_f32(const float* e, int hidden, int64_t num_nodes_out, const float* A1h,
                              const float* A2h, const float* A3h, int ld_node, const int32_t* in_ptr,
                              const int32_t* srt_src, const int32_t* out_ptr, const int32_t* out_pos,
                              const int32_t* out_dst, const float* h_in, int ld_h, float* h_out, int norm_kind,
                              const float* norm_scale, const float* norm_shift, void* stream);

int gnnome_build_node_records(const int32_t* in_ptr, const int32_t* srt_src, const int32_t* out_ptr, const int32_t* out_pos,
                              const int32_t* out_dst, int64_t num_nodes, int32_t* records, void* stream);
int gnnome_debug_node_records(const int32_t* records);

int gnnome_node_aggregate_range_f32(const float* e, int hidden, int64_t num_nodes_out, int64_t node_begin, int64_t node_end,
                                    const float* A1h, const float* A2h, const float* A3h, int ld_node, const int32_t* in_ptr,
                                    const int32_t* srt_src, const int32_t* out_ptr, const int32_t* out_pos,
                                    const int32_t* out_dst, const float* h_in, int ld_h, float* h_out, int norm_kind,
                                    const float* norm_scale, const float* norm_shift, void* stream);

int gnnome_stream_schedule_sizes(int64_t num_nodes, int64_t num_edges, int rows_per_step, int64_t* steps_capacity_host,
                                 size_t* scratch_bytes_host);
int gnnome_build_stream_schedule(int64_t num_nodes, int64_t num_edges, const int32_t* in_ptr, const int32_t* srt_src,
                                 const int32_t* out_ptr, const int32_t* out_pos, const int32_t* out_dst, int num_chunks,
                                 int rows_per_step, int num_slots, int32_t* chunk_node, int32_t* chunk_steps, int32_t* steps,
                                 uint8_t* edge_meta, int32_t* node_pend, int32_t* pend_nodes, int32_t* counters, void* scratch,
                                 size_t scratch_bytes, void* stream);
int gnnome_node_aggregate_stream_f32(const float* e, int hidden, int64_t num_nodes, int64_t num_edges, const float* A1h, const float* A2h,
                                     const float* A3h, int ld_node, const int32_t* in_ptr, const int32_t* srt_src,
                                     const int32_t* out_ptr, const int32_t* out_pos, const int32_t* out_dst, const float* h_in,
                                     int ld_h, float* h_out, const float* norm_scale, const float* norm_shift, int num_chunks,
                                     int rows_per_step, int num_slots, const int32_t* chunk_node, const int32_t* chunk_steps,
                                     const int32_t* steps, const uint8_t* edge_meta, const int32_t* node_pend,
                                     const int32_t* pend_nodes, const int32_t* counters, int64_t num_pending, float* pend_rows,
                                     void* stream);

int gnnome_edge_score_f32(const float* e, int64_t num_edges, int hidden, int hidden_edge_scores,
                          const float* Ps, const float* Qd, int ld_node, const int32_t* srt_src,
                          const int32_t* srt_dst, const int32_t* srt_eid, const float* W1e, int ldw1,
                          const float* W2, const float* b2, const float* W3, const float* b3, float* logits,
                          float* z1_out , void* stream);

typedef struct gnnome_layer_params {
    const float* Wcat;
    const void* Wcat_planes;
    const float* bcat;
    const float* W3;
    const float* b3;
    const float* scale_e;
    const float* shift_e;
    const float* scale_h;
    const float* shift_h;
    int32_t norm_kind;
    int32_t reference_order;
} gnnome_layer_params;

typedef struct gnnome_model_params {
    int32_t hidden, hidden_ne, num_layers, score_hidden, node_features, edge_features;
    const float *node_W1, *node_b1, *node_W2, *node_b2;
    const float *edge_W1, *edge_b1, *edge_W2, *edge_b2;
    const gnnome_layer_params* layers_host;
    const float* W_nodes;
    const void* W_nodes_planes;
    const float* b_nodes;
    const float* W1e;
    int32_t ld_w1e, reserved;
    const float *W2, *b2, *W3, *b3;
} gnnome_model_params;

typedef struct gnnome_views {
    int64_t num_nodes, num_edges;
    const int32_t *in_ptr, *srt_src, *srt_dst, *srt_eid, *out_ptr, *out_pos, *out_dst;
    const int32_t* node_gather;
    int32_t transposed, reserved;
} gnnome_views;

int gnnome_debug_forward_events(void* gate_start, void* gate_stop, void* aggregate_start, void* aggregate_stop, int layer);
int gnnome_model_forward_workspace_bytes(int64_t num_nodes, int64_t num_edges, int hidden, int score_hidden, size_t* bytes_host);
int gnnome_model_forward_f32(const gnnome_model_params* params_host, const gnnome_views* views_host, const float* x, const float* e_raw,
                             float* logits, void* workspace, size_t workspace_bytes, void* stream);
typedef struct gnnome_forward_buffers {
    float* h[2];
    float* P;
    float* e[2];
    float* PQ;
} gnnome_forward_buffers;
int gnnome_model_forward_buffers_f32(const gnnome_model_params* params_host, const gnnome_views* views_host, const float* x, const float* e_raw,
                                     float* logits, const gnnome_forward_buffers* buffers_host, void* stream);


int gnnome_edge_gate_raw_f32(const float* e_in, float* x_out, int64_t num_edges, int hidden, const float* B1h,
                             const float* B2h, int ld_node, const int32_t* srt_src, const int32_t* srt_dst,
                             const float* W3, int ldw, void* stream);

int gnnome_edge_gate_raw_stats_rows(int hidden, int* rows_host);
int gnnome_edge_gate_raw_stats_f32(const float* e_in, float* x_out, int64_t num_edges, int hidden, const float* B1h,
                                   const float* B2h, int ld_node, const int32_t* srt_src, const int32_t* srt_dst,
                                   const float* W3, int ldw, const float* center, float* stats_partial, void* stream);
int gnnome_edge_gate_bn_f32(const float* e_in, float* e_out, float* x_out, int64_t num_edges, int hidden, const float* B1h,
                            const float* B2h, int ld_node, const int32_t* srt_src, const int32_t* srt_dst, const float* W3, int ldw,
                            const float* scale, const float* shift, void* stream);

int gnnome_node_aggregate_raw_f32(const float* e, int hidden, int64_t num_nodes, int mode, const float* A1h,
                                  const float* A2h, const float* A3h, int ld_node, const int32_t* in_ptr,
                                  const int32_t* srt_src, const int32_t* out_ptr, const int32_t* out_pos,
                                  const int32_t* out_dst, float* v_out, float* aux0, float* aux1, float* aux2,
                                  float* aux3, void* stream);

int gnnome_colsum_workspace_bytes(size_t* bytes_host);
int gnnome_colsum2_f32(const float* x, const float* y, int64_t rows, int hidden, const float* center, float* s1,
                       float* s2, void* workspace, size_t workspace_bytes, void* stream);

int gnnome_bn_relu_res_f32(const float* x, const float* scale, const float* shift, const float* res, int64_t rows,
                           int hidden, float* out, void* stream);

int gnnome_bn_bwd_stats_f32(const float* dy, const float* x, const float* scale, const float* shift,
                            const float* mean, int64_t rows, int hidden, float* s1, float* s2, void* workspace,
                            size_t workspace_bytes, void* stream);
int gnnome_bn_bwd_apply_f32(const float* dy, const float* x, const float* scale, const float* shift, int64_t rows,
                            int hidden, const float* a, const float* c1, const float* c2, const float* mean,
                            const float* rstd, float* dx, void* stream);

int gnnome_bn_bwd_apply_tables_f32(const float* dy, const float* x, const float* scale, const float* shift, int64_t rows, int hidden,
                                   const float* a, const float* c1, const float* c2, const float* mean, const float* rstd,
                                   const float* rdf, const float* hf, const float* rdb, const float* hb, float* dx, float* Tf, float* Uf,
                                   float* Tb, float* Ub, unsigned* amax_bits, void* stream);

int gnnome_ln_relu_res_f32(const float* x, const float* gamma, const float* beta, const float* res, int64_t rows, int hidden,
                           int norm_width, float* out, void* stream);
int gnnome_ln_bwd_f32(const float* dy, const float* x, const float* gamma, const float* beta, int64_t rows, int hidden, int norm_width,
                      float* dx, float* dbeta, float* dgamma, void* workspace, size_t workspace_bytes, void* stream);

int gnnome_mul23_f32(const float* a, const float* b, const float* c, int64_t count, float* o1, float* o2, void* stream);
int gnnome_add_f32(const float* a, const float* b, int64_t count, float* out, void* stream);
int gnnome_relu_bwd_f32(const float* dy, const float* y, int64_t count, float* dx, void* stream);

int gnnome_segment_sum_f32(const float* X, int width, const int32_t* ptr, const int32_t* pos, int64_t num_nodes,
                           float* out, int ld_out, void* stream);

int gnnome_segment_sum2_f32(const float* X, int width, const int32_t* in_ptr, const int32_t* out_ptr, const int32_t* out_pos,
                            int64_t num_nodes, float* out_in, int ld_in, float* out_out, int ld_out, void* stream);

int gnnome_wgrad_workspace_bytes(int64_t rows, int Ka, int Kb, size_t* bytes_host);
int gnnome_wgrad_f32(const float* A, int lda, int Ka, const float* B, int ldb, int Kb, int64_t rows, float* C, int ldc,
                     void* workspace, size_t workspace_bytes, void* stream);
int gnnome_wgrad_scaled_f32(const float* A, int lda, int Ka, const float* B, int ldb, int Kb, int64_t rows, const unsigned* amax_bits,
                            float* C, int ldc, void* workspace, size_t workspace_bytes, void* stream);
int gnnome_wgrad_blocks_scaled_f32(const float* const* A_blocks, int num_blocks, int block_width, int lda, const float* B, int ldb, int Kb,
                                   int64_t rows, const unsigned* amax_bits, float* C, int ldc, float* colsum, void* workspace,
                                   size_t workspace_bytes, void* stream);
int gnnome_linear_blocks_scaled_f32(const float* const* A_blocks, int num_blocks, int block_width, int64_t M, int lda, const float* W, int ldw,
                                    int Nout, const unsigned* amax_bits, float* C, int ldc, int accumulate, void* stream);
int gnnome_segment_sum2_amax_f32(const float* X, int width, const int32_t* in_ptr, const int32_t* out_ptr, const int32_t* out_pos,
                                 int64_t num_nodes, float* out_in, int ld_in, float* out_out, int ld_out, unsigned* amax_bits, void* stream);

int gnnome_wgrad_blocks_f32(const float* const* A_blocks, int num_blocks, int block_width, int lda, const float* B, int ldb,
                            int Kb, int64_t rows, float* C, int ldc, float* colsum, void* workspace, size_t workspace_bytes,
                            void* stream);

int gnnome_linear_blocks_f32(const float* const* A_blocks, int num_blocks, int block_width, int64_t M, int lda, const float* W,
                             int ldw, int Nout, float* C, int ldc, int accumulate, void* stream);

int gnnome_score_tail_bwd_f32(const float* z1, const float* dscore, const int32_t* srt_eid, int64_t num_edges,
                              int hidden_edge_scores, const float* W2, const float* b2, const float* W3, float* dz1,
                              float* dz2, float* u, void* stream);

int gnnome_agg_edge_bwd_f32(const float* e, int64_t num_edges, int hidden, const float* Tf, const float* Uf,
                            const float* Tb, const float* Ub, const float* A2h, const float* A3h, int ld_node,
                            const int32_t* srt_src, const int32_t* srt_dst, float* de, void* stream);

int gnnome_encode_hidden_f32(const float* in, int64_t rows, int in_features, const int32_t* gather, const float* W1,
                             const float* b1, int hidden_ne, float* t, void* stream);

int gnnome_gather_rows_f32(const float* in, int ld_in, const int32_t* idx, int64_t rows, int width, float* out,
                           int ld_out, void* stream);

int gnnome_scatter_add_rows_f32(const float* in, int ld_in, const int32_t* idx, int64_t rows, int width, float* out,
                                int ld_out, void* stream);

int gnnome_closure_workspace_bytes(size_t* bytes_host);

int gnnome_degree_features_f32(const int32_t* in_ptr, const int32_t* out_ptr, int64_t num_nodes, int reverse, float* x,
                               void* workspace, size_t workspace_bytes, void* stream);

int gnnome_edge_features_f32(const float* overlap_length, const float* overlap_similarity, int64_t num_edges, float* e,
                             void* workspace, size_t workspace_bytes, void* stream);

int gnnome_edge_loss_f32(const float* logits, const float* logits_rev, const float* labels, int64_t num_edges,
                         const float* pos_weight, float alpha, float grad_scale, float* loss, float* dlogits,
                         float* dlogits_rev, int64_t* tfpn, void* workspace, size_t workspace_bytes, void* stream);

int gnnome_bn_bwd_dgrad_f32(float* C, const float* X, int64_t rows, int64_t rows_once, int hidden, const float* scale, const float* shift,
                            const float* a, const float* c1, const float* c2, const float* mean, const float* rstd,
                            const float* W, int ldw, float* dxe, void* stream);
int gnnome_bn_bwd_dgrad_amax_f32(float* C, const float* X, int64_t rows, int64_t rows_once, int hidden, const float* scale, const float* shift,
                                 const float* a, const float* c1, const float* c2, const float* mean, const float* rstd,
                                 const float* W, int ldw, float* dxe, unsigned* amax_bits, void* stream);
int gnnome_bn_bwd_dgrad_out_f32(const float* C_in, float* C_out, const float* X, int64_t rows, int64_t rows_once, int hidden,
                                const float* scale, const float* shift, const float* a, const float* c1, const float* c2,
                                const float* mean, const float* rstd, const float* W, int ldw, float* dxe, void* stream);
int gnnome_bn_bwd_dgrad_out_amax_f32(const float* C_in, float* C_out, const float* X, int64_t rows, int64_t rows_once, int hidden,
                                     const float* scale, const float* shift, const float* a, const float* c1, const float* c2,
                                     const float* mean, const float* rstd, const float* W, int ldw, float* dxe, unsigned* amax_bits, void* stream);

int gnnome_agg_edge_bwd_stats_f32(const float* e, int64_t num_edges, int hidden, const float* Tf, const float* Uf,
                                  const float* Tb, const float* Ub, const float* A2h, const float* A3h, int ld_node,
                                  const int32_t* srt_src, const int32_t* srt_dst, float* de, const float* xe, const float* scale,
                                  const float* shift, const float* mean, float* s1, float* s2, void* workspace,
                                  size_t workspace_bytes, void* stream);

int gnnome_agg_bwd_fused_f32(const float* e, int64_t num_nodes, int64_t num_edges, int hidden, const float* Tf, const float* Uf,
                             const float* Tb, const float* Ub, const float* A2h, const float* A3h, int ld_node, const int32_t* in_ptr,
                             const int32_t* srt_src, const int32_t* out_ptr, const int32_t* out_pos, const int32_t* out_dst, float* de,
                             const float* xe, const float* scale, const float* shift, const float* mean, float* sum_in, float* sum_out,
                             float* s1, float* s2, unsigned* amax_bits, void* workspace, size_t workspace_bytes, void* stream);

int gnnome_bn_train_finish_f32(const float* d1, const float* d2, const float* center, int64_t rows, int hidden, const float* gamma,
                               const float* beta, float* running_mean, float* running_var, int64_t* num_batches_tracked,
                               float momentum, float eps, int updates, float* mean, float* rstd, float* scale, float* shift,
                               void* stream);
// ... 102 lines not shown
```

Measured before the change: 243.8 million.

## Precompute folded edge-encoder weights once and add a direct 256-thread enc16 kernel

The W3·encW2 fold for the first layer's encoded edge gate is now computed once at engine preparation and passed through a new folded entry point, so the per-forward fold kernel launch is skipped. A new k_edge_gate_enc16_direct kernel, which uses 256 threads, DPP quad gathers and software-pipelined loads, is added but only runs when the experiment tuning knob is 16 or 17. Shared quad_transpose and frag_col helpers move to common.h. The fold result is cached across calls, which is valid only while the weights stay fixed.

```diff
diff --git a/gnnome_amd/_lib.py b/gnnome_amd/_lib.py
--- a/gnnome_amd/_lib.py
+++ b/gnnome_amd/_lib.py
@@ -25,6 +25,8 @@
     "gnnome_linear_planes_route": [_l, _i, _i, _i],
     "gnnome_edge_gate_f32": [_p, _p, _l, _i, _p, _p, _i, _p, _p, _p, _i, _i, _p, _p, _p],
     "gnnome_edge_gate_encode_f32": [_p, _p, _p, _p, _p, _p, _p, _l, _i, _p, _p, _i, _p, _p, _p, _i, _p, _p, _p],
+    "gnnome_fold_edge_encoder_f32": [_p, _i, _p, _p, _i, _p, _p, _p],
+    "gnnome_edge_gate_encode_folded_f32": [_p, _p, _p, _p, _p, _p, _p, _l, _i, _p, _p, _i, _p, _p, _p, _i, _p, _p, _p, _p, _p],
     "gnnome_linear_ref_f32": [_p, _l, _i, _i, _p, _i, _p, _i, _p, _i, _p],
     "gnnome_edge_gate_ref_f32": [_p, _p, _l, _i, _p, _p, _i, _p, _p, _p, _i, _p, _p, _p, _p, _p, _p, _p, _p, _p, _p],
     "gnnome_node_aggregate_f32": [_p, _i, _l, _p, _p, _p, _i, _p, _p, _p, _p, _p, _p, _i, _p, _i, _p, _p, _p],
@@ -119,7 +121,7 @@
     "gnnome_gfa_pack": [_p, _l, _p, _p, _l, _p, _l, _p],
 }
 
-ABI_VERSION = 21
+ABI_VERSION = 22
 
 
 class LayerParams(ctypes.Structure):
@@ -131,7 +133,8 @@
     _fields_ = ([(n, ctypes.c_int32) for n in ("hidden", "hidden_ne", "num_layers", "score_hidden", "node_features", "edge_features")]
                 + [(n, _p) for n in ("node_W1", "node_b1", "node_W2", "node_b2", "edge_W1", "edge_b1", "edge_W2", "edge_b2")]
                 + [("layers_host", ctypes.POINTER(LayerParams)), ("W_nodes", _p), ("W_nodes_planes", _p), ("b_nodes", _p), ("W1e", _p),
-                   ("ld_w1e", ctypes.c_int32), ("reserved", ctypes.c_int32), ("W2", _p), ("b2", _p), ("W3", _p), ("b3", _p)])
+                   ("ld_w1e", ctypes.c_int32), ("reserved", ctypes.c_int32), ("W2", _p), ("b2", _p), ("W3", _p), ("b3", _p),
+                   ("edge_W23", _p), ("edge_b23", _p)])
 
 
 class Views(ctypes.Structure):
diff --git a/gnnome_amd/csrc/common.h b/gnnome_amd/csrc/common.h
--- a/gnnome_amd/csrc/common.h
+++ b/gnnome_amd/csrc/common.h
@@ -127,6 +127,24 @@
     return base + bid / kXcds;
 }
 
+__host__ __device__ constexpr int frag_col(int i) { return 16 * ((i >> 2) & 1) + 4 * (i >> 3) + (i & 3); }
+
+__device__ __forceinline__ float quad_xor1(float v) { return __int_as_float(__builtin_amdgcn_mov_dpp(__float_as_int(v), 0xB1, 0xF, 0xF, true)); }
+__device__ __forceinline__ float quad_xor2(float v) { return __int_as_float(__builtin_amdgcn_mov_dpp(__float_as_int(v), 0x4E, 0xF, 0xF, true)); }
+__device__ __forceinline__ void quad_transpose(f32x4& E0, f32x4& E1, f32x4& E2, f32x4& E3, int lane) {
+    const bool hi2 = lane & 2, hi1 = lane & 1;
+#define GN_SWAP(X, Y, COND, XOR)                       \
+    _Pragma("unroll") for (int t = 0; t < 4; ++t) {    \
+        const float x = X[t], y = Y[t];                \
+        const float py = XOR(y), px = XOR(x);          \
+        X[t] = COND ? py : x;                          \
+        Y[t] = COND ? y : px;                          \
+    }
+    GN_SWAP(E0, E2, hi2, quad_xor2) GN_SWAP(E1, E3, hi2, quad_xor2)
+    GN_SWAP(E0, E1, hi1, quad_xor1) GN_SWAP(E2, E3, hi1, quad_xor1)
+#undef GN_SWAP
+}
+
 __device__ __forceinline__ float sigmoidf_(float x) { return __builtin_amdgcn_rcpf(1.0f + __expf(-x)); }
 
 __device__ __forceinline__ float relu_keep_nan(float t) { return t < 0.f ? 0.f : t; }
diff --git a/gnnome_amd/csrc/edge_gate.hip b/gnnome_amd/csrc/edge_gate.hip
--- a/gnnome_amd/csrc/edge_gate.hip
+++ b/gnnome_amd/csrc/edge_gate.hip
@@ -665,11 +665,10 @@
     return gate_bn_impl(e_in, e_out, x_out, num_edges, hidden, B1h, B2h, ld_node, srt_src, srt_dst, W3, ldw, scale, shift, stream, true);
 }
 
-extern "C" int gnnome_edge_gate_encode_f32(const float* e_raw, const int32_t* srt_eid, const float* encW1, const float* encb1,
-                                           const float* encW2, const float* encb2, float* e_out, int64_t num_edges, int hidden,
-                                           const float* B1h, const float* B2h, int ld_node, const int32_t* srt_src,
-                                           const int32_t* srt_dst, const float* W3, int ldw, const float* norm_scale,
-                                           const float* norm_shift, void* stream) {
+static int edge_gate_encode_impl(const float* e_raw, const int32_t* srt_eid, const float* encW1, const float* encb1, const float* encW2,
+                                 const float* encb2, float* e_out, int64_t num_edges, int hidden, const float* B1h, const float* B2h,
+                                 int ld_node, const int32_t* srt_src, const int32_t* srt_dst, const float* W3, int ldw,
+                                 const float* norm_scale, const float* norm_shift, const float* W23, const float* b23, void* stream) {
     using namespace gnnome;
     GN_REQUIRE(num_edges >= 0, "edge_gate_encode: negative edge count");
     if (num_edges == 0) return GNNOME_OK;
@@ -679,7 +678,8 @@
                "edge_gate_encode: hidden=%d not in {64,128,256 (default kernels)}", hidden);
     GN_REQUIRE(ld_node % 4 == 0 && ldw % 4 == 0 && ((uintptr_t)B1h % 16 == 0) && ((uintptr_t)B2h % 16 == 0) && ((uintptr_t)W3 % 16 == 0),
                "edge_gate_encode: alignment");
-    const GateEnc enc = {e_raw, srt_eid, encW1, encb1, encW2, encb2};
+    GN_REQUIRE((W23 == nullptr) == (b23 == nullptr) && (uintptr_t)W23 % 16 == 0, "edge_gate_encode: W23 and b23 come together, W23 16-byte aligned");
+    const GateEnc enc = {e_raw, srt_eid, encW1, encb1, encW2, encb2, hidden == 128 ? W23 : nullptr, hidden == 128 ? b23 : nullptr};
     hipStream_t s = (hipStream_t)stream;
     if (hidden == 256) {
         GN_REQUIRE((uintptr_t)e_out % 16 == 0, "edge_gate_encode: e_out must be 16-byte aligned");
@@ -698,3 +698,21 @@
         return launch_gate_ws<4, 1>(nullptr, e_out, num_edges, B1h, B2h, ld_node, srt_src, srt_dst, W3, ldw, norm_scale, norm_shift, s, &enc);
     return launch_gate_ws<2, 2>(nullptr, e_out, num_edges, B1h, B2h, ld_node, srt_src, srt_dst, W3, ldw, norm_scale, norm_shift, s, &enc);
 }
+
+extern "C" int gnnome_edge_gate_encode_f32(const float* e_raw, const int32_t* srt_eid, const float* encW1, const float* encb1,
+                                           const float* encW2, const float* encb2, float* e_out, int64_t num_edges, int hidden,
+                                           const float* B1h, const float* B2h, int ld_node, const int32_t* srt_src,
+                                           const int32_t* srt_dst, const float* W3, int ldw, const float* norm_scale,
+                                           const float* norm_shift, void* stream) {
+    return edge_gate_encode_impl(e_raw, srt_eid, encW1, encb1, encW2, encb2, e_out, num_edges, hidden, B1h, B2h, ld_node, srt_src, srt_dst, W3, ldw,
+                                 norm_scale, norm_shift, nullptr, nullptr, stream);
+}
+
+extern "C" int gnnome_edge_gate_encode_folded_f32(const float* e_raw, const int32_t* srt_eid, const float* encW1, const float* encb1,
+                                                  const float* encW2, const float* encb2, float* e_out, int64_t num_edges, int hidden,
+                                                  const float* B1h, const float* B2h, int ld_node, const int32_t* srt_src,
+                                                  const int32_t* srt_dst, const float* W3, int ldw, const float* norm_scale,
+                                                  const float* norm_shift, const float* W23, const float* b23, void* stream) {
+    return edge_gate_encode_impl(e_raw, srt_eid, encW1, encb1, encW2, encb2, e_out, num_edges, hidden, B1h, B2h, ld_node, srt_src, srt_dst, W3, ldw,
+                                 norm_scale, norm_shift, W23, b23, stream);
+}
diff --git a/gnnome_amd/csrc/edge_gate_bf.hip b/gnnome_amd/csrc/edge_gate_bf.hip
--- a/gnnome_amd/csrc/edge_gate_bf.hip
+++ b/gnnome_amd/csrc/edge_gate_bf.hip
@@ -923,6 +923,145 @@
     }
 }
 
+__device__ __forceinline__ int quad_lane(int v, int r) {
+    return r == 0 ? __builtin_amdgcn_mov_dpp(v, 0x00, 0xF, 0xF, true) : r == 1 ? __builtin_amdgcn_mov_dpp(v, 0x55, 0xF, 0xF, true)
+         : r == 2 ? __builtin_amdgcn_mov_dpp(v, 0xAA, 0xF, 0xF, true) : __builtin_amdgcn_mov_dpp(v, 0xFF, 0xF, 0xF, true);
+}
+
+template <int WPS>
+__global__ __launch_bounds__(256, WPS) void k_edge_gate_enc16_direct(GateBfArgs a) {
+    constexpr int H = 128, TM = 32;
+    __shared__ __attribute__((aligned(16))) float w1s[32], b1s[16];
+    const int tid = threadIdx.x, lane = tid & 63;
+    const int cb = __builtin_amdgcn_readfirstlane(tid >> 6);
+    const int j = lane & 31, half = lane >> 5, g4 = lane & 28;
+    const int per_xcd = gridDim.x / kXcds;
+    const int first = (int)(blockIdx.x % kXcds) * per_xcd + (int)(blockIdx.x / kXcds);
+    const int stride = (int)gridDim.x;
+    const int n = first < a.num_tiles ? (a.num_tiles - first + stride - 1) / stride : 0;
+    if (n <= 0) return;
+    auto tile_of = [&](int r) { return first + min(r, n - 1) * stride; };
+    auto tile_valid = [&](int r) { return (int)min((int64_t)TM, a.E - (int64_t)tile_of(r) * TM); };
+    if (tid < 32) w1s[tid] = a.enc.W1[tid];
+    if (tid >= 64 && tid < 80) b1s[tid - 64] = a.enc.b1[tid - 64];
+    __syncthreads();
+
+    uint4 u1, u2, u3, v1, v2, v3;
+    {
+        const int col = 32 * cb + frag_col(j);
+        const float* p = a.enc.W23 + col * 16 + 8 * half;
+        split3(*reinterpret_cast<const f32x4*>(p), *reinterpret_cast<const f32x4*>(p + 4), u1, u2, u3);
+        const float* q = a.enc.W2 + col * 16 + 8 * half;
+        split3(*reinterpret_cast<const f32x4*>(q), *reinterpret_cast<const f32x4*>(q + 4), v1, v2, v3);
+    }
+    const int c0 = 32 * cb + 16 * half + 4 * (lane & 3);
+    f32x4 sc4, sh4, bx4, be4;
+#pragma unroll
+    for (int t = 0; t < 4; ++t) {
+        sc4[t] = a.scale[c0 + t];
+        sh4[t] = a.shift[c0 + t];
+        bx4[t] = a.enc.b23[c0 + t];
+        be4[t] = a.enc.b2[c0 + t];
+    }
+    const float* B1c = a.B1h + c0;
+    const float* B2c = a.B2h + c0;
+
+    int si, di, eid;
+    f32x4 g1[4], g2[4];
+    float raw0, raw1;
+    auto issue_indices = [&](int r) {
+        const int64_t row = (int64_t)tile_of(r) * TM + min(j, tile_valid(r) - 1);
+        asm volatile("global_load_dword %0, %1, off" : "=v"(si) : "v"(a.srt_src + row) : "memory");
+        asm volatile("global_load_dword %0, %1, off" : "=v"(di) : "v"(a.srt_dst + row) : "memory");
+        asm volatile("global_load_dword %0, %1, off" : "=v"(eid) : "v"(a.enc.srt_eid + row) : "memory");
+    };
+    auto issue_gathers = [&]() {
+        const float* pr = a.enc.e_raw + 2 * (int64_t)eid;
+        const float* p1[4];
+        const float* p2[4];
+#pragma unroll
+        for (int q = 0; q < 4; ++q) {
+            p1[q] = B1c + (int64_t)quad_lane(si, q) * a.ldn;
+            p2[q] = B2c + (int64_t)quad_lane(di, q) * a.ldn;
+        }
+        asm volatile("global_load_dword %0, %1, off" : "=v"(raw0) : "v"(pr) : "memory");
+        asm volatile("global_load_dword %0, %1, off offset:4" : "=v"(raw1) : "v"(pr) : "memory");
+#pragma unroll
+        for (int q = 0; q < 4; ++q) {
+            asm volatile("global_load_dwordx4 %0, %1, off" : "=v"(g1[q]) : "v"(p1[q]) : "memory");
+            asm volatile("global_load_dwordx4 %0, %1, off" : "=v"(g2[q]) : "v"(p2[q]) : "memory");
+        }
+    };
+    issue_indices(0);
+    asm volatile("s_waitcnt vmcnt(0)" : "+v"(si), "+v"(di), "+v"(eid)::"memory");
+    issue_gathers();
+    issue_indices(1);
+    asm volatile("s_waitcnt vmcnt(0)" ::: "memory");
+    for (int r = 0; r < n; ++r) {
+        asm volatile("s_waitcnt vmcnt(4)"
+                     : "+v"(g1[0]), "+v"(g1[1]), "+v"(g1[2]), "+v"(g1[3]), "+v"(g2[0]), "+v"(g2[1]), "+v"(g2[2]), "+v"(g2[3]), "+v"(raw0), "+v"(raw1),
+                       "+v"(si), "+v"(di), "+v"(eid)::"memory");
+        f32x4 tl, th, gk[4];
+        {
+            const f32x4* w = reinterpret_cast<const f32x4*>(w1s + 16 * half);
+            const f32x4 wa = w[0], wb = w[1], wc = w[2], wd = w[3];
+            const f32x4 ba = *reinterpret_cast<const f32x4*>(b1s + 8 * half), bb = *reinterpret_cast<const f32x4*>(b1s + 8 * half + 4);
+            tl[0] = fmaxf(__builtin_fmaf(raw1, wa[1], raw0 * wa[0]) + ba[0], 0.f);
+            tl[1] = fmaxf(__builtin_fmaf(raw1, wa[3], raw0 * wa[2]) + ba[1], 0.f);
+            tl[2] = fmaxf(__builtin_fmaf(raw1, wb[1], raw0 * wb[0]) + ba[2], 0.f);
+            tl[3] = fmaxf(__builtin_fmaf(raw1, wb[3], raw0 * wb[2]) + ba[3], 0.f);
+            th[0] = fmaxf(__builtin_fmaf(raw1, wc[1], raw0 * wc[0]) + bb[0], 0.f);
+            th[1] = fmaxf(__builtin_fmaf(raw1, wc[3], raw0 * wc[2]) + bb[1], 0.f);
+            th[2] = fmaxf(__builtin_fmaf(raw1, wd[1], raw0 * wd[0]) + bb[2], 0.f);
+            th[3] = fmaxf(__builtin_fmaf(raw1, wd[3], raw0 * wd[2]) + bb[3], 0.f);
+        }
+#pragma unroll
+        for (int q = 0; q < 4; ++q) gk[q] = g1[q] + g2[q];
+        asm volatile("" : "+v"(gk[0]), "+v"(gk[1]), "+v"(gk[2]), "+v"(gk[3]), "+v"(tl), "+v"(th)::"memory");
+        issue_gathers();
+        issue_indices(r + 2);
+        __builtin_amdgcn_sched_barrier(0);
+        uint4 c1, c2, c3;
+        split3(tl, th, c1, c2, c3);
+        f32x16 ax, ae;
+#pragma unroll
+        for (int i = 0; i < 16; ++i) ax[i] = ae[i] = 0.f;
+        ax = __builtin_amdgcn_mfma_f32_32x32x16_bf16(as_bf(u1), as_bf(c3), ax, 0, 0, 0);
+        ae = __builtin_amdgcn_mfma_f32_32x32x16_bf16(as_bf(v1), as_bf(c3), ae, 0, 0, 0);
+        ax = __builtin_amdgcn_mfma_f32_32x32x16_bf16(as_bf(u3), as_bf(c1), ax, 0, 0, 0);
+        ae = __builtin_amdgcn_mfma_f32_32x32x16_bf16(as_bf(v3), as_bf(c1), ae, 0, 0, 0);
+        ax = __builtin_amdgcn_mfma_f32_32x32x16_bf16(as_bf(u2), as_bf(c2), ax, 0, 0, 0);
+        ae = __builtin_amdgcn_mfma_f32_32x32x16_bf16(as_bf(v2), as_bf(c2), ae, 0, 0, 0);
+        ax = __builtin_amdgcn_mfma_f32_32x32x16_bf16(as_bf(u1), as_bf(c2), ax, 0, 0, 0);
+        ae = __builtin_amdgcn_mfma_f32_32x32x16_bf16(as_bf(v1), as_bf(c2), ae, 0, 0, 0);
+        ax = __builtin_amdgcn_mfma_f32_32x32x16_bf16(as_bf(u2), as_bf(c1), ax, 0, 0, 0);
+        ae = __builtin_amdgcn_mfma_f32_32x32x16_bf16(as_bf(v2), as_bf(c1), ae, 0, 0, 0);
+        ax = __builtin_amdgcn_mfma_f32_32x32x16_bf16(as_bf(u1), as_bf(c1), ax, 0, 0, 0);
+        ae = __builtin_amdgcn_mfma_f32_32x32x16_bf16(as_bf(v1), as_bf(c1), ae, 0, 0, 0);
+        f32x4 X[4], E0[4];
+#pragma unroll
+        for (int q = 0; q < 4; ++q)
+#pragma unroll
+            for (int t = 0; t < 4; ++t) {
+                X[q][t] = ax[4 * q + t];
+                E0[q][t] = ae[4 * q + t];
+            }
+        quad_transpose(X[0], X[1], X[2], X[3], lane);
+        quad_transpose(E0[0], E0[1], E0[2], E0[3], lane);
+        const int last = tile_valid(r) - 1;
+        float* out = a.e_out + (int64_t)tile_of(r) * TM * H + c0;
+#pragma unroll
+        for (int q = 0; q < 4; ++q) {
+            const f32x4 x = X[q] + bx4, e0 = E0[q] + be4;
+            f32x4 y;
+#pragma unroll
+            for (int t = 0; t < 4; ++t) y[t] = fmaxf((x[t] + gk[q][t]) * sc4[t] + sh4[t], 0.f) + e0[t];
+            *reinterpret_cast<f32x4*>(out + min(g4 + q, last) * H) = y;
+        }
+    }
+    asm volatile("s_waitcnt vmcnt(0)" ::: "memory");
+}
+
 struct EncFoldScratch {
     float* w23 = nullptr;
 };
@@ -934,16 +1073,25 @@
     GN_REQUIRE(tiles < (1ll << 31), "edge_gate: too many tiles");
     a.num_tiles = (int)tiles;
     a.xp = tuning(kTuneGateExperiment);
-    int dev = 0;
-    GN_HIP(hipGetDevice(&dev));
-    GN_REQUIRE(dev >= 0 && dev < 16, "edge_gate_encode: device index %d", dev);
-    if (!g_enc_fold[dev].w23) GN_HIP(hipMalloc(&g_enc_fold[dev].w23, sizeof(float) * (128 * 16 + 128)));
-    float* w23 = g_enc_fold[dev].w23;
-    hipLaunchKernelGGL(k_fold_encoder, dim3((128 * 17 + 3) / 4), dim3(256), 0, s, a.W3, a.ldw, a.enc.W2, a.enc.b2, 128, w23, w23 + 128 * 16);
-    GN_LAUNCH_CHECK();
-    a.enc.W23 = w23;
-    a.enc.b23 = w23 + 128 * 16;
-    hipLaunchKernelGGL(k_edge_gate_enc16, dim3(persistent_grid()), dim3(640), 0, s, a);
+    if (a.enc.W23 == nullptr) {
+        int dev = 0;
+        GN_HIP(hipGetDevice(&dev));
+        GN_REQUIRE(dev >= 0 && dev < 16, "edge_gate_encode: device index %d", dev);
+        if (!g_enc_fold[dev].w23) GN_HIP(hipMalloc(&g_enc_fold[dev].w23, sizeof(float) * (128 * 16 + 128)));
+        float* w23 = g_enc_fold[dev].w23;
+        hipLaunchKernelGGL(k_fold_encoder, dim3((128 * 17 + 3) / 4), dim3(256), 0, s, a.W3, a.ldw, a.enc.W2, a.enc.b2, 128, w23, w23 + 128 * 16);
+        GN_LAUNCH_CHECK();
+        a.enc.W23 = w23;
+        a.enc.b23 = w23 + 128 * 16;
+    }
+    GN_REQUIRE((uintptr_t)a.e_out % 16 == 0 && (uintptr_t)a.enc.W2 % 16 == 0, "edge_gate_encode: e_out and encW2 must be 16-byte aligned");
+    if (a.xp == 16) {
+        hipLaunchKernelGGL(k_edge_gate_enc16_direct<3>, dim3(3 * persistent_grid()), dim3(256), 0, s, a);
+    } else if (a.xp == 17) {
+        hipLaunchKernelGGL(k_edge_gate_enc16_direct<2>, dim3(2 * persistent_grid()), dim3(256), 0, s, a);
+    } else {
+        hipLaunchKernelGGL(k_edge_gate_enc16, dim3(persistent_grid()), dim3(640), 0, s, a);
+    }
     GN_LAUNCH_CHECK();
     return GNNOME_OK;
 }
@@ -1018,6 +1166,16 @@
 
 }
 
+extern "C" int gnnome_fold_edge_encoder_f32(const float* W3, int ldw, const float* encW2, const float* encb2, int hidden, float* W23, float* b23,
+                                            void* stream) {
+    using namespace gnnome;
+    GN_REQUIRE(W3 && encW2 && encb2 && W23 && b23, "fold_edge_encoder: null pointer");
+    GN_REQUIRE((hidden == 64 || hidden == 128 || hidden == 256) && ldw >= hidden, "fold_edge_encoder: hidden=%d not in {64,128,256} or ldw=%d below it", hidden, ldw);
+    hipLaunchKernelGGL(k_fold_encoder, dim3((hidden * 17 + 3) / 4), dim3(256), 0, (hipStream_t)stream, W3, ldw, encW2, encb2, hidden, W23, b23);
+    GN_LAUNCH_CHECK();
+    return GNNOME_OK;
+}
+
 extern "C" int gnnome_debug_gate_profile(void* counters) {
     gnnome::g_gate_prof = (long long*)counters;
     return GNNOME_OK;
diff --git a/gnnome_amd/csrc/model_forward.cpp b/gnnome_amd/csrc/model_forward.cpp
--- a/gnnome_amd/csrc/model_forward.cpp
+++ b/gnnome_amd/csrc/model_forward.cpp
@@ -154,8 +154,8 @@
                                             e ? nullptr : m->edge_W2, e ? nullptr : m->edge_b2, stream));
             e = out;
         } else if (e == nullptr) {
-            GN_TRY(gnnome_edge_gate_encode_f32(e_raw, g->srt_eid, m->edge_W1, m->edge_b1, m->edge_W2, m->edge_b2, eb[0], E, H, B1, B2, 5 * H, g->srt_src,
-                                               g->srt_dst, lw.W3, H, lw.scale_e, lw.shift_e, stream));
+            GN_TRY(gnnome_edge_gate_encode_folded_f32(e_raw, g->srt_eid, m->edge_W1, m->edge_b1, m->edge_W2, m->edge_b2, eb[0], E, H, B1, B2, 5 * H,
+                                                      g->srt_src, g->srt_dst, lw.W3, H, lw.scale_e, lw.shift_e, m->edge_W23, m->edge_b23, stream));
             e = eb[0];
         } else if (H == 256 && lw.norm_kind == GNNOME_NORM_AFFINE) {
             float* out = e == eb[0] ? eb[1] : eb[0];
diff --git a/gnnome_amd/csrc/node_project.hip b/gnnome_amd/csrc/node_project.hip
--- a/gnnome_amd/csrc/node_project.hip
+++ b/gnnome_amd/csrc/node_project.hip
@@ -31,22 +31,6 @@
         asm volatile("s_waitcnt vmcnt(0)" : "+v"(r[0]), "+v"(r[1]), "+v"(r[2]), "+v"(r[3]), "+v"(r[4]), "+v"(r[5]), "+v"(r[6]), "+v"(r[7])::"memory");
     else
         asm volatile("" : "+v"(r[0]), "+v"(r[1]), "+v"(r[2]), "+v"(r[3]), "+v"(r[4]), "+v"(r[5]), "+v"(r[6]), "+v"(r[7])::"memory");
-}
-
-__device__ __forceinline__ float quad_xor1(float v) { return __int_as_float(__builtin_amdgcn_mov_dpp(__float_as_int(v), 0xB1, 0xF, 0xF, true)); }
-__device__ __forceinline__ float quad_xor2(float v) { return __int_as_float(__builtin_amdgcn_mov_dpp(__float_as_int(v), 0x4E, 0xF, 0xF, true)); }
-__device__ __forceinline__ void quad_transpose(f32x4& E0, f32x4& E1, f32x4& E2, f32x4& E3, int lane) {
-    const bool hi2 = lane & 2, hi1 = lane & 1;
-#define GN_SWAP(X, Y, COND, XOR)                       \
-    _Pragma("unroll") for (int t = 0; t < 4; ++t) {    \
-        const float x = X[t], y = Y[t];                \
-        const float py = XOR(y), px = XOR(x);          \
-        X[t] = COND ? py : x;                          \
-        Y[t] = COND ? y : px;                          \
-    }
-    GN_SWAP(E0, E2, hi2, quad_xor2) GN_SWAP(E1, E3, hi2, quad_xor2)
-    GN_SWAP(E0, E1, hi1, quad_xor1) GN_SWAP(E2, E3, hi1, quad_xor1)
-#undef GN_SWAP
 }
 
 __device__ __forceinline__ void split8(const f32x4 lo, const f32x4 hi, h8_t& p1, h8_t& p2) {
@@ -65,8 +49,6 @@
 }
 
 }
-
-__host__ __device__ constexpr int frag_col(int i) { return 16 * ((i >> 2) & 1) + 4 * (i >> 3) + (i & 3); }
 
 __global__ __launch_bounds__(256) void k_weight_planes(const float* __restrict__ W, int ldw, int Nout, int K, uint4* __restrict__ planes) {
     const int t = blockIdx.x * 256 + threadIdx.x;
diff --git a/gnnome_amd/engine.py b/gnnome_amd/engine.py
--- a/gnnome_amd/engine.py
+++ b/gnnome_amd/engine.py
@@ -49,6 +49,11 @@
                                                _pad(model.linear2_edge.weight.detach(), H, ne), _pad(model.linear2_edge.bias.detach(), H)))
         self.layers = [prepare_layer(conv, device, arithmetic) for conv in model.gnn.convs]
         self.predictor = prepare_predictor(model.predictor, device)
+        self.enc_fold = None
+        fold = getattr(hip_ops, "fold_edge_encoder", None)
+        if (fold is not None and H == 128 and self.layers and not self.layers[0].ref and self.layers[0].norm == NORM_AFFINE
+                and self.layers[0].W3.is_cuda and tuple(self.enc_edge[0].shape) == (16, 2)):
+            self.enc_fold = fold(self.layers[0].W3, self.enc_edge[2], self.enc_edge[3])
         weights = [t for lw in self.layers for t in (lw.Wcat, lw.W3)] + [self.predictor["_W1"], self.predictor["W2"]]
         amax = max((float(t.abs().max()) if t.numel() else 0.0) for t in weights) if weights else 0.0
         self.force_bf16x6 = not (amax < hip_ops_fp16_max())
@@ -238,8 +243,10 @@
 
 def gate(ops, lw, views, e, B1, B2, raw_edges=None, scratch=None):
     if lw.ref:
-        return ops.edge_gate_ref(e, B1, B2, views, lw.W3, lw.b3, lw.scale_e, lw.shift_e, raw_edges=raw_edges)
+        return ops.edge_gate_ref(e, B1, B2, views, lw.W3, lw.b3, lw.scale_e, lw.shift_e, raw_edges=None if raw_edges is None else tuple(raw_edges[:2]))
     if e is None:
+        if len(raw_edges) > 2 and raw_edges[2] is not None:
+            return ops.edge_gate_encode(raw_edges[0], raw_edges[1], B1, B2, views, lw.W3, lw.scale_e, lw.shift_e, fold=raw_edges[2])
         return ops.edge_gate_encode(raw_edges[0], raw_edges[1], B1, B2, views, lw.W3, lw.scale_e, lw.shift_e)
     return gate_update(ops, lw, views, e, B1, B2, scratch)
 
@@ -347,7 +354,8 @@
         then = None
         if pipelined:
             then = layer_projection(ops, prep.layers[i + 1]) if i + 1 < len(prep.layers) else predictor_projection(ops, prep.predictor)
-        h, e, P = layer_step(ops, lw, views, h, e, n_out=n_own, raw_edges=(e_raw, prep.enc_edge), scratch=scratch, P=P, then=then)
+        fold = getattr(prep, "enc_fold", None) if (i == 0 and getattr(ops, "fold_edge_encoder", None) is not None) else None
+        h, e, P = layer_step(ops, lw, views, h, e, n_out=n_own, raw_edges=(e_raw, prep.enc_edge, fold), scratch=scratch, P=P, then=then)
     if exchange is not None:
         h = exchange(h)
     if logits is None:
diff --git a/gnnome_amd/ops.py b/gnnome_amd/ops.py
--- a/gnnome_amd/ops.py
+++ b/gnnome_amd/ops.py
@@ -299,7 +299,8 @@
 
     def __init__(self, prep):
         pw = prep.predictor
-        self.keep = [prep.enc_node, prep.enc_edge, prep.layers, pw]
+        fold = getattr(prep, "enc_fold", None)
+        self.keep = [prep.enc_node, prep.enc_edge, prep.layers, pw, fold]
         n = len(prep.layers)
         self.layers = (_lib.LayerParams * max(n, 1))()
         for lp, lw in zip(self.layers, prep.layers):
@@ -325,6 +326,7 @@
         m.W_nodes, m.W_nodes_planes, m.b_nodes = _dptr(pw["W_nodes"]), _dptr(pw.get("planes")), _dptr(pw["b_nodes"])
         m.W1e, m.ld_w1e = _dptr(W1e), W1e.stride(0)
         m.W2, m.b2, m.W3, m.b3 = (_dptr(pw[k]) for k in ("W2", "b2", "W3", "b3"))
+        m.edge_W23, m.edge_b23 = (_dptr(fold[0]), _dptr(fold[1])) if fold is not None else (None, None)
 
 
 def _views_block(views):
@@ -501,16 +503,35 @@
             and norm_kind == NORM_AFFINE and e_raw.shape[0] > 0 and B1h.stride(0) % 4 == 0 and B1h.data_ptr() % 16 == 0)
 
 
-def edge_gate_encode(e_raw, enc, B1h, B2h, views, W3, scale, shift):
+def fold_edge_encoder(W3, W2, b2):
+    lib = _lib.load()
+    W3, ldw = _rows(W3, "fold_edge_encoder.W3")
+    W2, b2 = _dense(W2, "fold_edge_encoder.W2"), _dense(b2, "fold_edge_encoder.b2")
+    H = W3.shape[0]
+    W23 = torch.empty((H, 16), dtype=torch.float32, device=W3.device)
+    b23 = torch.empty(H, dtype=torch.float32, device=W3.device)
+    with _on(W3.device):
+        _lib.check(lib.gnnome_fold_edge_encoder_f32(_ptr(W3), ldw, _ptr(W2), _ptr(b2), H, _ptr(W23), _ptr(b23), _stream(W3.device)), "fold_edge_encoder_f32")
+    return W23, b23
+
+
+def edge_gate_encode(e_raw, enc, B1h, B2h, views, W3, scale, shift, fold=None, out=None):
     lib = _lib.load()
     e_raw = _dense(e_raw, "edge_gate_encode.e_raw")
     B1h, ldn = _rows(B1h, "edge_gate_encode.B1h")
     B2h, _ = _rows(B2h, "edge_gate_encode.B2h")
     W3, ldw = _rows(W3, "edge_gate_encode.W3")
     E, H = views.num_edges, W3.shape[0]
-    out = torch.empty((E, H), dtype=torch.float32, device=e_raw.device)
+    if out is None:
+        out = torch.empty((E, H), dtype=torch.float32, device=e_raw.device)
     W1, b1, W2, b2 = enc
     with _on(e_raw.device):
+        if fold is not None:
+            _lib.check(lib.gnnome_edge_gate_encode_folded_f32(_ptr(e_raw), _ptr(views.srt_eid), _ptr(W1), _ptr(b1), _ptr(W2), _ptr(b2),
+                                                              _ptr(out), E, H, _ptr(B1h), _ptr(B2h), ldn, _ptr(views.srt_src),
+                                                              _ptr(views.srt_dst), _ptr(W3), ldw, _ptr(scale), _ptr(shift),
+                                                              _ptr(fold[0]), _ptr(fold[1]), _stream(e_raw.device)), "edge_gate_encode_folded_f32")
+            return out
         _lib.check(lib.gnnome_edge_gate_encode_f32(_ptr(e_raw), _ptr(views.srt_eid), _ptr(W1), _ptr(b1), _ptr(W2), _ptr(b2),
                                                    _ptr(out), E, H, _ptr(B1h), _ptr(B2h), ldn, _ptr(views.srt_src),
                                                    _ptr(views.srt_dst), _ptr(W3), ldw, _ptr(scale), _ptr(shift),
diff --git a/include/gnnome_hip.h b/include/gnnome_hip.h
--- a/include/gnnome_hip.h
+++ b/include/gnnome_hip.h
@@ -8,7 +8,7 @@
 extern "C" {
 #endif
 
-#define GNNOME_ABI_VERSION 21
+#define GNNOME_ABI_VERSION 22
 
 #define GNNOME_OK 0
 #define GNNOME_EINVAL (-1)
@@ -56,6 +56,13 @@
                                 const float* B1h, const float* B2h, int ld_node, const int32_t* srt_src,
                                 const int32_t* srt_dst, const float* W3, int ldw, const float* norm_scale,
                                 const float* norm_shift, void* stream);
+int gnnome_fold_edge_encoder_f32(const float* W3, int ldw, const float* encW2, const float* encb2, int hidden, float* W23, float* b23,
+                                 void* stream);
+int gnnome_edge_gate_encode_folded_f32(const float* e_raw, const int32_t* srt_eid, const float* encW1, const float* encb1,
+                                       const float* encW2, const float* encb2, float* e_out, int64_t num_edges, int hidden,
+                                       const float* B1h, const float* B2h, int ld_node, const int32_t* srt_src,
+                                       const int32_t* srt_dst, const float* W3, int ldw, const float* norm_scale,
+                                       const float* norm_shift, const float* W23, const float* b23, void* stream);
 
 int gnnome_linear_ref_f32(const float* A, int64_t M, int K, int lda, const float* W, int ldw, const float* bias, int Nout,
                           float* C, int ldc, void* stream);
@@ -128,6 +135,7 @@
     const float* W1e;
     int32_t ld_w1e, reserved;
     const float *W2, *b2, *W3, *b3;
+    const float *edge_W23, *edge_b23;
 } gnnome_model_params;
 
 typedef struct gnnome_views {
```

Measured after the change: 243.8 million, median of 2. About the same (-0.0%).
